# haileys/mixlab

Hardware: AMD Instinct MI355X
Metric: audio_ch_mixed_per_sec (higher is better)
Workload: dtype f32 (f64 intermediates); 1 GPU; 1024-channel Mixer + EqThree + Envelope chain (Trigger->Envelope; noise->EqThree->StereoPanner->Amplifier->Mixer), 48000 Hz f32; strips=1024, gates=toggle every 30 ticks, phase k mod 60, applied between ticks inside the batch, eq_mode=exact order: speculative time-parallel kernel, verified bit-exact, parallelism=strips sharded x1, ticks_policy=one GPU

## Files before the change

include/mixlab_gpu.h:

```cpp
#ifndef MIXLAB_GPU_H
#define MIXLAB_GPU_H

#include <stddef.h>
#include <stdint.h>

#ifdef __cplusplus
extern "C" {
#endif

#define MX_ABI_VERSION 4u

enum {
    MX_OK = 0,
    MX_ERR_INVALID = -1,
    MX_ERR_TYPE = -2,
    MX_ERR_DEVICE = -3,
    MX_ERR_NOMEM = -4,
    MX_ERR_INTERNAL = -5,
    MX_ERR_FULL = -6
};

typedef enum { MX_DISCONNECTED = 0, MX_MONO = 1, MX_STEREO = 2, MX_VIDEO = 3 } mx_line;

enum {
// ... 13 lines not shown
    MX_KIND_SOURCE_VIDEO = 13,
    MX_KIND_VIDEO_TO_RGBA = 14,
    MX_KIND_FIR = 15,
    MX_KIND_RESAMPLE = 16,
    MX_KIND_MONITOR = 17,
    MX_KIND_OUTPUT_DEVICE = 18,
    MX_KIND_COUNT = 19
};
#define MX_PROFILE_KINDS 18

enum { MX_WAVE_ON = 0, MX_WAVE_OFF = 1, MX_WAVE_SINE = 2, MX_WAVE_SQUARE = 3, MX_WAVE_TRIANGLE = 4, MX_WAVE_SAW = 5 };

typedef struct { double gain_db; double fader; uint8_t cue; uint8_t _pad[7]; } mx_mixer_channel_params;
typedef struct { double gain_lo_db, gain_mid_db, gain_hi_db; } mx_eq_three_params;
typedef struct { double attack_ms, decay_ms, sustain_amplitude, release_ms; } mx_envelope_params;
typedef struct { double amplitude, mod_depth; } mx_amplifier_params;
typedef struct { double freq; uint32_t waveform; uint32_t _pad; } mx_oscillator_params;
typedef struct { double freq_lo, freq_hi; } mx_fm_sine_params;
typedef struct { uint32_t gate_open; } mx_trigger_params;
typedef struct { int32_t a, b;  double fader; } mx_video_mixer_params;
typedef struct { int32_t use_matrix; int32_t matrix_q12[12]; } mx_video_to_rgba_params;
typedef struct { uint32_t width, height; } mx_monitor_params;
typedef struct { uint32_t width, height, queue_depth, _pad; } mx_monitor_params_ex;
typedef struct { uint32_t channels; int32_t left, right; uint32_t _pad; } mx_output_device_params;
typedef struct { uint32_t n_taps; uint32_t _pad;  } mx_fir_params;
typedef struct { uint32_t up, down, taps_per_phase, _pad;  } mx_resample_params;

typedef struct { uint32_t kind; uint32_t params_len; const void* params; } mx_node;
typedef struct { uint32_t src_node, src_port, dst_node, dst_port; } mx_edge;

#define MX_FLAG_EQ_EXACT 1u
#define MX_FLAG_EQ_FAST 4u
#define MX_FLAG_FP_CONTRACT 16u

#define MX_FLAG_OVERLAP_TAIL 8u
#define MX_FLAG_NO_FUSE 2u

typedef struct {
    uint32_t sample_rate;
    uint32_t ticks_per_second;
    uint32_t max_ticks_per_run;
    uint32_t flags;
    int32_t device;
    int32_t _pad;
    void* stream;
} mx_graph_opts;

typedef struct mx_graph mx_graph;

const char* mx_last_error(void);
uint32_t mx_abi_version(void);
int mx_device_count(void);

int mx_graph_build(const mx_node* nodes, size_t n_nodes, const mx_edge* edges, size_t n_edges,
                   const mx_graph_opts* opts, mx_graph** out);
void mx_graph_destroy(mx_graph* g);

int mx_graph_samples_per_tick(const mx_graph* g, size_t* spt);
int mx_graph_run_order(const mx_graph* g, uint32_t* order, size_t cap, size_t* n);

int mx_graph_stream(mx_graph* g, void** stream);
int mx_graph_tail_stream(mx_graph* g, void** stream);

int mx_graph_update_params(mx_graph* g, uint32_t node, const void* params, size_t params_len);

typedef struct { uint32_t node; uint32_t tick_in_run; const void* params; size_t params_len; } mx_param_event;
int mx_graph_schedule_params(mx_graph* g, uint32_t node, uint32_t tick_in_run, const void* params, size_t params_len);
int mx_graph_schedule_params_batch(mx_graph* g, const mx_param_event* events, size_t n_events);

int mx_graph_eq_spec_stats(mx_graph* g, uint64_t* chunks_run, uint64_t* chunks_repaired);
int mx_graph_eq_repair_stats(mx_graph* g, uint64_t out[8]);
int mx_graph_debug_eq_records(mx_graph* g, void** device_records, size_t* bytes);
int mx_graph_debug_tail_releases(mx_graph* g, uint64_t* gated, uint64_t* at_once);
#define MX_EQ_LAUNCH_NONE 0u
#define MX_EQ_LAUNCH_SEQUENTIAL 1u
#define MX_EQ_LAUNCH_DIRECT 2u
#define MX_EQ_LAUNCH_TILED 3u
#define MX_EQ_LAUNCH_RAGGED_TICK 4u
#define MX_EQ_LAUNCH_CONTROL_TILE 5u
#define MX_EQ_LAUNCH_SCAN 6u
int mx_graph_debug_eq_launch(mx_graph* g, uint32_t out[5]);
int mx_graph_debug_eq_env_rows(mx_graph* g, uint32_t* rows);
int mx_graph_debug_eq_lean(mx_graph* g, uint32_t* lean);
typedef struct mx_plan_node {
    int32_t pos;
    int32_t level, group;
    uint32_t slot;
    int32_t sub_key;
    uint32_t dom_num, dom_den, in_dom_num, in_dom_den;
    uint32_t elided;
    int32_t owner;
    int32_t fuse_pan, fuse_amp, fuse_trigger, fuse_env;
    uint32_t n_out;
    uint8_t out_elided[4];
    uint8_t out_dup[4];
    uint64_t out_off[4];
    uint64_t out_off2[4];
} mx_plan_node;
typedef struct mx_plan_info {
    uint64_t n_order, n_groups;
    uint64_t slab_floats;
    uint64_t zero_off, zero_floats;
    int32_t tail_first_group;
    uint32_t tail_ports;
    uint32_t tail_auto;
    uint32_t has_video;
} mx_plan_info;
int mx_graph_debug_plan(const mx_node* nodes, size_t n_nodes, const mx_edge* edges, size_t n_edges, const mx_graph_opts* opts,
                        uint32_t overlap_auto, size_t cap_frames, mx_plan_node* nodes_out, mx_plan_info* info);

int mx_graph_write_source(mx_graph* g, uint32_t node, const float* host_samples, size_t n_ticks);
int mx_graph_bind_source_device(mx_graph* g, uint32_t node, const void* device_ptr);

int mx_graph_run_ticks(mx_graph* g, uint64_t first_tick, uint32_t n_ticks);
int mx_graph_sync(mx_graph* g);

int mx_graph_read_output(mx_graph* g, uint32_t node, uint32_t port, float* host_samples, size_t n_ticks);
int mx_graph_read_output_window(mx_graph* g, uint32_t node, uint32_t port, float* host_samples, size_t first_tick_in_run, size_t n_ticks);
int mx_graph_read_output_i16(mx_graph* g, uint32_t node, uint32_t port, int16_t* host_samples, size_t n_ticks);
int mx_graph_write_source_i16(mx_graph* g, uint32_t node, const int16_t* host_samples, size_t n_ticks);

int mx_graph_output_device_ptr(mx_graph* g, uint32_t node, uint32_t port, void** device_ptr, size_t* floats_per_tick);

typedef struct { uint8_t clip, clip_status, lag_status, changed; uint32_t channels; } mx_audio_out_tick;
int mx_graph_read_audio_out(mx_graph* g, uint32_t node, uint32_t first_tick_in_run, uint32_t n_ticks, float* samples, size_t samples_cap,
                            mx_audio_out_tick* ticks, size_t* n_samples);
int mx_graph_audio_out_lag(mx_graph* g, uint32_t node);

typedef struct { uint32_t node, port; } mx_port_ref;
typedef struct { uint32_t hold_ticks; float release; } mx_meter_params;
typedef struct {
    float    peak[2];
    float    hold[2];
    double   sum_sq[2];
    uint32_t over[2];
    uint32_t frames;
    uint32_t channels;
} mx_meter_tick;
int mx_graph_set_meters(mx_graph* g, const mx_port_ref* ports, size_t n, const mx_meter_params* params);
int mx_graph_read_meters(mx_graph* g, uint32_t first_tick_in_run, uint32_t n_ticks, mx_meter_tick* dst, size_t cap);

typedef struct {
    uint32_t        n_fft;
    uint32_t        n_bands;
    const uint16_t* edges;
} mx_spectrum_params;
int mx_graph_set_spectra(mx_graph* g, const mx_port_ref* ports, size_t n, const mx_spectrum_params* params);
int mx_graph_read_spectra(mx_graph* g, uint32_t first_tick_in_run, uint32_t n_ticks, float* dst, size_t cap);
int mx_spectrum_tables(uint32_t n_fft, float* window, float* twiddle_re, float* twiddle_im);

typedef struct { uint32_t momentary_ticks; uint32_t short_ticks; } mx_loudness_params;
typedef struct {
    double   ksq[2];
    double   momentary_sq;
    double   short_sq;
    float    true_peak[2];
    uint32_t frames;
    uint32_t channels;
} mx_loudness_tick;
int mx_graph_set_loudness(mx_graph* g, const mx_port_ref* ports, size_t n, const mx_loudness_params* params);
int mx_graph_read_loudness(mx_graph* g, uint32_t first_tick_in_run, uint32_t n_ticks, mx_loudness_tick* dst, size_t cap);
int mx_loudness_tables(double rate, uint32_t frames_per_tick, double* biquads, double* carry, float* interp);
int mx_loudness_gate(const double* block_sq, const uint32_t* block_frames, size_t n_blocks, double* lufs_integrated, size_t* blocks_kept);

typedef struct { uint32_t window_ticks , grid , zoom_log2 , hop ; } mx_stereo_params;
typedef struct {
// ... 415 lines not shown
```

mixlab_amd/abi.py:

```python
from __future__ import annotations

import ctypes as C
import pathlib

import numpy as np

_PKG = pathlib.Path(__file__).resolve().parent
LIB_PATH = _PKG / "libmixlab_gpu.so"

if not LIB_PATH.exists():
    raise ImportError(
        f"{LIB_PATH} is missing: build it with `python -m mixlab_amd.build` (hipcc, gfx950). "
        "mixlab_amd has no CPU fallback."
    )

lib = C.CDLL(str(LIB_PATH))

MX_OK, MX_ERR_INVALID, MX_ERR_TYPE, MX_ERR_DEVICE, MX_ERR_NOMEM, MX_ERR_INTERNAL, MX_ERR_FULL = 0, -1, -2, -3, -4, -5, -6
MX_DISCONNECTED, MX_MONO, MX_STEREO, MX_VIDEO = 0, 1, 2, 3
(KIND_AMPLIFIER, KIND_ENVELOPE, KIND_EQ_THREE, KIND_FM_SINE, KIND_MIXER, KIND_OSCILLATOR, KIND_PLOTTER,
 KIND_STEREO_PANNER, KIND_STEREO_SPLITTER, KIND_TRIGGER, KIND_VIDEO_MIXER, KIND_SOURCE_MONO,
 KIND_SOURCE_STEREO, KIND_SOURCE_VIDEO, KIND_VIDEO_TO_RGBA, KIND_FIR, KIND_RESAMPLE, KIND_MONITOR, KIND_OUTPUT_DEVICE, KIND_COUNT) = range(20)
PROFILE_KINDS = 18
KIND_NAMES = ["amplifier", "envelope", "eq_three", "fm_sine", "mixer", "oscillator", "plotter", "stereo_panner",
# ... 9 lines not shown


class MixerChannelParams(C.Structure):
    _fields_ = [("gain_db", C.c_double), ("fader", C.c_double), ("cue", C.c_uint8), ("_pad", C.c_uint8 * 7)]


class EqThreeParams(C.Structure):
    _fields_ = [("gain_lo_db", C.c_double), ("gain_mid_db", C.c_double), ("gain_hi_db", C.c_double)]


class EnvelopeParams(C.Structure):
    _fields_ = [("attack_ms", C.c_double), ("decay_ms", C.c_double), ("sustain_amplitude", C.c_double), ("release_ms", C.c_double)]


class AmplifierParams(C.Structure):
    _fields_ = [("amplitude", C.c_double), ("mod_depth", C.c_double)]


class OscillatorParams(C.Structure):
    _fields_ = [("freq", C.c_double), ("waveform", C.c_uint32), ("_pad", C.c_uint32)]


class FmSineParams(C.Structure):
    _fields_ = [("freq_lo", C.c_double), ("freq_hi", C.c_double)]


class TriggerParams(C.Structure):
    _fields_ = [("gate_open", C.c_uint32)]


class Node(C.Structure):
    _fields_ = [("kind", C.c_uint32), ("params_len", C.c_uint32), ("params", C.c_void_p)]


class Edge(C.Structure):
    _fields_ = [("src_node", C.c_uint32), ("src_port", C.c_uint32), ("dst_node", C.c_uint32), ("dst_port", C.c_uint32)]


class GraphOpts(C.Structure):
    _fields_ = [("sample_rate", C.c_uint32), ("ticks_per_second", C.c_uint32), ("max_ticks_per_run", C.c_uint32),
                ("flags", C.c_uint32), ("device", C.c_int32), ("_pad", C.c_int32), ("stream", C.c_void_p)]


class Frame(C.Structure):
    _fields_ = [("width", C.c_uint32), ("height", C.c_uint32), ("data", C.c_void_p * 3), ("stride", C.c_int32 * 3),
                ("dur_num", C.c_int64), ("dur_den", C.c_int64), ("off_num", C.c_int64), ("off_den", C.c_int64)]


class Input(C.Structure):
    _fields_ = [("kind", C.c_int), ("samples", C.c_void_p), ("len", C.c_size_t), ("video", C.c_void_p)]


class Output(C.Structure):
    _fields_ = [("kind", C.c_int), ("samples", C.c_void_p), ("len", C.c_size_t), ("video", C.c_void_p), ("video_present", C.c_int)]


def _proto(name, restype, *argtypes):
    fn = getattr(lib, name)
    fn.restype = restype
    fn.argtypes = list(argtypes)
    return fn


_proto("mx_last_error", C.c_char_p)
_proto("mx_abi_version", C.c_uint32)
_proto("mx_device_count", C.c_int)
_proto("mx_graph_build", C.c_int, C.POINTER(Node), C.c_size_t, C.POINTER(Edge), C.c_size_t, C.POINTER(GraphOpts), C.POINTER(C.c_void_p))
_proto("mx_graph_destroy", None, C.c_void_p)
_proto("mx_graph_samples_per_tick", C.c_int, C.c_void_p, C.POINTER(C.c_size_t))
_proto("mx_graph_run_order", C.c_int, C.c_void_p, C.POINTER(C.c_uint32), C.c_size_t, C.POINTER(C.c_size_t))
_proto("mx_graph_update_params", C.c_int, C.c_void_p, C.c_uint32, C.c_void_p, C.c_size_t)
class ParamEvent(C.Structure):
    _fields_ = [("node", C.c_uint32), ("tick_in_run", C.c_uint32), ("params", C.c_void_p), ("params_len", C.c_size_t)]


_proto("mx_graph_schedule_params", C.c_int, C.c_void_p, C.c_uint32, C.c_uint32, C.c_void_p, C.c_size_t)
_proto("mx_graph_schedule_params_batch", C.c_int, C.c_void_p, C.POINTER(ParamEvent), C.c_size_t)
_proto("mx_graph_eq_spec_stats", C.c_int, C.c_void_p, C.POINTER(C.c_uint64), C.POINTER(C.c_uint64))
_proto("mx_graph_debug_eq_records", C.c_int, C.c_void_p, C.POINTER(C.c_void_p), C.POINTER(C.c_size_t))
_proto("mx_graph_debug_tail_releases", C.c_int, C.c_void_p, C.POINTER(C.c_uint64), C.POINTER(C.c_uint64))
_proto("mx_graph_debug_eq_launch", C.c_int, C.c_void_p, C.POINTER(C.c_uint32))
_proto("mx_graph_debug_eq_env_rows", C.c_int, C.c_void_p, C.POINTER(C.c_uint32))
_proto("mx_graph_debug_eq_lean", C.c_int, C.c_void_p, C.POINTER(C.c_uint32))
_proto("mx_graph_eq_repair_stats", C.c_int, C.c_void_p, C.POINTER(C.c_uint64))
PLAN_NONE = 2**64 - 1


class PlanNode(C.Structure):
    _fields_ = [("pos", C.c_int32), ("level", C.c_int32), ("group", C.c_int32), ("slot", C.c_uint32), ("sub_key", C.c_int32),
                ("dom_num", C.c_uint32), ("dom_den", C.c_uint32), ("in_dom_num", C.c_uint32), ("in_dom_den", C.c_uint32),
                ("elided", C.c_uint32), ("owner", C.c_int32),
                ("fuse_pan", C.c_int32), ("fuse_amp", C.c_int32), ("fuse_trigger", C.c_int32), ("fuse_env", C.c_int32),
                ("n_out", C.c_uint32), ("out_elided", C.c_uint8 * 4), ("out_dup", C.c_uint8 * 4),
                ("out_off", C.c_uint64 * 4), ("out_off2", C.c_uint64 * 4)]


class PlanInfo(C.Structure):
    _fields_ = [("n_order", C.c_uint64), ("n_groups", C.c_uint64), ("slab_floats", C.c_uint64), ("zero_off", C.c_uint64), ("zero_floats", C.c_uint64),
                ("tail_first_group", C.c_int32), ("tail_ports", C.c_uint32), ("tail_auto", C.c_uint32), ("has_video", C.c_uint32)]


_proto("mx_graph_debug_plan", C.c_int, C.POINTER(Node), C.c_size_t, C.POINTER(Edge), C.c_size_t, C.POINTER(GraphOpts), C.c_uint32, C.c_size_t,
       C.POINTER(PlanNode), C.POINTER(PlanInfo))
_proto("mx_graph_write_source", C.c_int, C.c_void_p, C.c_uint32, C.c_void_p, C.c_size_t)
_proto("mx_graph_bind_source_device", C.c_int, C.c_void_p, C.c_uint32, C.c_void_p)
_proto("mx_graph_run_ticks", C.c_int, C.c_void_p, C.c_uint64, C.c_uint32)
_proto("mx_graph_sync", C.c_int, C.c_void_p)
_proto("mx_graph_read_output", C.c_int, C.c_void_p, C.c_uint32, C.c_uint32, C.c_void_p, C.c_size_t)
_proto("mx_graph_read_output_window", C.c_int, C.c_void_p, C.c_uint32, C.c_uint32, C.c_void_p, C.c_size_t, C.c_size_t)
_proto("mx_graph_read_output_i16", C.c_int, C.c_void_p, C.c_uint32, C.c_uint32, C.c_void_p, C.c_size_t)
_proto("mx_graph_write_source_i16", C.c_int, C.c_void_p, C.c_uint32, C.c_void_p, C.c_size_t)
_proto("mx_graph_output_device_ptr", C.c_int, C.c_void_p, C.c_uint32, C.c_uint32, C.POINTER(C.c_void_p), C.POINTER(C.c_size_t))
_proto("mx_graph_tail_stream", C.c_int, C.c_void_p, C.POINTER(C.c_void_p))
_proto("mx_graph_stream", C.c_int, C.c_void_p, C.POINTER(C.c_void_p))
_proto("mx_graph_read_plotter", C.c_int, C.c_void_p, C.c_uint32, C.c_uint32, C.c_void_p, C.c_void_p, C.POINTER(C.c_int))
class OutputDeviceParams(C.Structure):
    _fields_ = [("channels", C.c_uint32), ("left", C.c_int32), ("right", C.c_int32), ("_pad", C.c_uint32)]


class AudioOutTick(C.Structure):
    _fields_ = [("clip", C.c_uint8), ("clip_status", C.c_uint8), ("lag_status", C.c_uint8), ("changed", C.c_uint8), ("channels", C.c_uint32)]


AUDIO_OUT_TICK_DTYPE = np.dtype([("clip", np.uint8), ("clip_status", np.uint8), ("lag_status", np.uint8), ("changed", np.uint8), ("channels", np.uint32)])
_proto("mx_graph_read_audio_out", C.c_int, C.c_void_p, C.c_uint32, C.c_uint32, C.c_uint32, C.c_void_p, C.c_size_t, C.c_void_p, C.POINTER(C.c_size_t))
_proto("mx_graph_audio_out_lag", C.c_int, C.c_void_p, C.c_uint32)
class PortRef(C.Structure):
    _fields_ = [("node", C.c_uint32), ("port", C.c_uint32)]


class MeterParams(C.Structure):
    _fields_ = [("hold_ticks", C.c_uint32), ("release", C.c_float)]


METER_TICK_DTYPE = np.dtype({"names": ["peak", "hold", "sum_sq", "over", "frames", "channels"],
                             "formats": [(np.float32, 2), (np.float32, 2), (np.float64, 2), (np.uint32, 2), np.uint32, np.uint32],
                             "offsets": [0, 8, 16, 32, 40, 44], "itemsize": 48})
_proto("mx_graph_set_meters", C.c_int, C.c_void_p, C.c_void_p, C.c_size_t, C.c_void_p)
_proto("mx_graph_read_meters", C.c_int, C.c_void_p, C.c_uint32, C.c_uint32, C.c_void_p, C.c_size_t)
class SpectrumParams(C.Structure):
    _fields_ = [("n_fft", C.c_uint32), ("n_bands", C.c_uint32), ("edges", C.POINTER(C.c_uint16))]


_proto("mx_graph_set_spectra", C.c_int, C.c_void_p, C.c_void_p, C.c_size_t, C.c_void_p)
_proto("mx_graph_read_spectra", C.c_int, C.c_void_p, C.c_uint32, C.c_uint32, C.c_void_p, C.c_size_t)
_proto("mx_spectrum_tables", C.c_int, C.c_uint32, C.c_void_p, C.c_void_p, C.c_void_p)
class LoudnessParams(C.Structure):
    _fields_ = [("momentary_ticks", C.c_uint32), ("short_ticks", C.c_uint32)]


LOUDNESS_TICK_DTYPE = np.dtype({"names": ["ksq", "momentary_sq", "short_sq", "true_peak", "frames", "channels"],
                                "formats": [(np.float64, 2), np.float64, np.float64, (np.float32, 2), np.uint32, np.uint32],
                                "offsets": [0, 16, 24, 32, 40, 44], "itemsize": 48})
_proto("mx_graph_set_loudness", C.c_int, C.c_void_p, C.c_void_p, C.c_size_t, C.c_void_p)
_proto("mx_graph_read_loudness", C.c_int, C.c_void_p, C.c_uint32, C.c_uint32, C.c_void_p, C.c_size_t)
_proto("mx_loudness_tables", C.c_int, C.c_double, C.c_uint32, C.c_void_p, C.c_void_p, C.c_void_p)
_proto("mx_loudness_gate", C.c_int, C.c_void_p, C.c_void_p, C.c_size_t, C.POINTER(C.c_double), C.POINTER(C.c_size_t))
class StereoParams(C.Structure):
    _fields_ = [("window_ticks", C.c_uint32), ("grid", C.c_uint32), ("zoom_log2", C.c_uint32), ("hop", C.c_uint32)]


STEREO_TICK_DTYPE = np.dtype({"names": ["sum_ll", "sum_rr", "sum_lr", "win_ll", "win_rr", "win_lr", "frames", "nonfinite"],
                              "formats": [np.float64] * 6 + [np.uint32] * 2,
                              "offsets": [0, 8, 16, 24, 32, 40, 48, 52], "itemsize": 56})
_proto("mx_graph_set_stereo", C.c_int, C.c_void_p, C.c_void_p, C.c_size_t, C.c_void_p)
_proto("mx_graph_read_stereo", C.c_int, C.c_void_p, C.c_uint32, C.c_uint32, C.c_void_p, C.c_size_t)
# ... 453 lines not shown
    e_arr = (Edge * max(1, len(edges)))()
    for i, e in enumerate(edges):
        e_arr[i] = Edge(*e)
    return n_arr, e_arr, keep


def debug_plan(nodes, edges, sample_rate=44100, ticks_per_second=60, max_ticks_per_run=1, flags=0, overlap_auto=1, cap_frames=0):
    n_arr, e_arr, _keep = _graph_arrays(nodes, edges)
    opts = GraphOpts(sample_rate, ticks_per_second, max_ticks_per_run, flags, -1, 0, None)
    out = (PlanNode * max(1, len(nodes)))()
    info = PlanInfo()
    check(lib.mx_graph_debug_plan(n_arr, len(nodes), e_arr, len(edges), C.byref(opts), overlap_auto, cap_frames, out, C.byref(info)))
    return list(out[: len(nodes)]), info


class Graph:

    def __init__(self, nodes, edges, sample_rate=44100, ticks_per_second=60, max_ticks_per_run=1, flags=0,
                 device=-1, stream=None):
        self._h = C.c_void_p()
        n_arr, e_arr, self._keep = _graph_arrays(nodes, edges)
        opts = GraphOpts(sample_rate, ticks_per_second, max_ticks_per_run, flags, device, 0, stream)
        check(lib.mx_graph_build(n_arr, len(nodes), e_arr, len(edges), C.byref(opts), C.byref(self._h)))
        spt = C.c_size_t()
        check(lib.mx_graph_samples_per_tick(self._h, C.byref(spt)))
        self.spt = spt.value
        self.max_ticks = max_ticks_per_run
        self.n_nodes = len(nodes)

    def close(self):
        if getattr(self, "_h", None) is not None and self._h.value:
            lib.mx_graph_destroy(self._h)
            self._h = C.c_void_p()

    def __del__(self):
        try:
            self.close()
        except Exception:
            pass

    def run_order(self):
        n = C.c_size_t()
        arr = (C.c_uint32 * max(1, self.n_nodes))()
        check(lib.mx_graph_run_order(self._h, arr, self.n_nodes, C.byref(n)))
        return list(arr[: n.value])

    def update_params(self, node, params):
        blob = params_bytes(params)
        check(lib.mx_graph_update_params(self._h, node, blob, len(blob)))

    def schedule_params(self, node, tick_in_run: int, params):
        blob = params_bytes(params)
        check(lib.mx_graph_schedule_params(self._h, node, tick_in_run, blob, len(blob)))

    def schedule_params_batch(self, events: "C.Array", n: int | None = None):
        check(lib.mx_graph_schedule_params_batch(self._h, events, len(events) if n is None else n))

    def eq_repair_stats(self) -> dict:
        v = (C.c_uint64 * 8)()
        check(lib.mx_graph_eq_repair_stats(self._h, v))
        keys = ("chunks_run", "chunks_repaired", "settled_by_comparison", "walk_steps_16", "fill_steps_16", "island_rounds", "in_order_walks", "nan_fills")
        return {k: int(x) for k, x in zip(keys, v)}

    def debug_tail_releases(self):
        a, b = C.c_uint64(), C.c_uint64()
        check(lib.mx_graph_debug_tail_releases(self._h, C.byref(a), C.byref(b)))
        return a.value, b.value

    def debug_eq_launch(self) -> dict:
        v = (C.c_uint32 * 5)()
        check(lib.mx_graph_debug_eq_launch(self._h, v))
        return {"form": EQ_LAUNCH.get(v[0], str(v[0])), "super_block": int(v[1]), "n_chunks": int(v[2]), "chunk": int(v[3]), "warm": int(v[4])}

    def debug_eq_env_rows(self) -> bool:
        v = C.c_uint32()
        check(lib.mx_graph_debug_eq_env_rows(self._h, C.byref(v)))
        return bool(v.value)

    def debug_eq_lean(self) -> dict:
        v = C.c_uint32()
        check(lib.mx_graph_debug_eq_lean(self._h, C.byref(v)))
        return {"untracked": bool(v.value & 1), "unity": bool(v.value & 2)}

    def debug_eq_records(self):
        p, n = C.c_void_p(), C.c_size_t()
        check(lib.mx_graph_debug_eq_records(self._h, C.byref(p), C.byref(n)))
        return p.value, n.value

    def eq_spec_stats(self):
        a, b = C.c_uint64(), C.c_uint64()
        check(lib.mx_graph_eq_spec_stats(self._h, C.byref(a), C.byref(b)))
        return a.value, b.value

    def write_source(self, node, samples: np.ndarray, n_ticks: int):
        a = np.ascontiguousarray(samples, dtype=np.float32)
        check(lib.mx_graph_write_source(self._h, node, a.ctypes.data_as(C.c_void_p), n_ticks))

    def bind_source_device(self, node, device_ptr: int):
        check(lib.mx_graph_bind_source_device(self._h, node, C.c_void_p(device_ptr)))

    def run_ticks(self, first_tick: int, n_ticks: int = 1):
        check(lib.mx_graph_run_ticks(self._h, first_tick, n_ticks))

    def sync(self):
        check(lib.mx_graph_sync(self._h))

    def read_output(self, node, port, n_ticks: int, stereo: bool, rate=(1, 1)) -> np.ndarray:
        out = np.empty(n_ticks * (self.spt * rate[0] // rate[1]) * (2 if stereo else 1), dtype=np.float32)
        check(lib.mx_graph_read_output(self._h, node, port, out.ctypes.data_as(C.c_void_p), n_ticks))
        return out

    def read_output_window(self, node, port, first_tick: int, n_ticks: int, stereo: bool) -> np.ndarray:
        out = np.empty(n_ticks * self.spt * (2 if stereo else 1), dtype=np.float32)
        check(lib.mx_graph_read_output_window(self._h, node, port, out.ctypes.data_as(C.c_void_p), first_tick, n_ticks))
        return out

    def read_audio_out(self, node, first_tick: int, n_ticks: int):
        n = C.c_size_t(0)
        check(lib.mx_graph_read_audio_out(self._h, node, first_tick, n_ticks, None, 0, None, C.byref(n)))
        samples = np.empty(n.value, dtype=np.float32)
        ticks = np.empty(n_ticks, dtype=AUDIO_OUT_TICK_DTYPE)
        check(lib.mx_graph_read_audio_out(self._h, node, first_tick, n_ticks, samples.ctypes.data_as(C.c_void_p), n.value,
                                          ticks.ctypes.data_as(C.c_void_p), C.byref(n)))
        return samples, ticks

    def audio_out_lag(self, node):
        check(lib.mx_graph_audio_out_lag(self._h, node))

    def set_meters(self, ports, params=MeterParams(0, 1.0)):
        ports = list(ports)
        if isinstance(params, MeterParams):
            params = [params] * len(ports)
        pa = (PortRef * max(1, len(ports)))(*[PortRef(int(n), int(p)) for (n, p) in ports])
        pr = (MeterParams * max(1, len(ports)))(*[MeterParams(q.hold_ticks, q.release) for q in params])
        check(lib.mx_graph_set_meters(self._h, pa, len(ports), pr))
        self._n_meters = len(ports)

    def read_meters(self, first_tick: int, n_ticks: int) -> np.ndarray:
        n = getattr(self, "_n_meters", 0)
        out = np.zeros((n_ticks, n), dtype=METER_TICK_DTYPE)
        check(lib.mx_graph_read_meters(self._h, first_tick, n_ticks, out.ctypes.data_as(C.c_void_p), out.size))
        return out

    def set_spectra(self, ports, n_fft: int = 2048, edges=None):
        ports = list(ports)
        if not ports:
            check(lib.mx_graph_set_spectra(self._h, None, 0, None))
            self._spectra = (0, 0)
            return
        e = np.ascontiguousarray(edges, dtype=np.uint16)
        if e.ndim != 1 or e.size < 2 or not np.array_equal(e, np.asarray(edges)):
            raise ValueError("edges: at least two bin indices that fit 16 bits")
        pa = (PortRef * len(ports))(*[PortRef(int(n), int(p)) for (n, p) in ports])
        pr = SpectrumParams(int(n_fft), e.size - 1, e.ctypes.data_as(C.POINTER(C.c_uint16)))
        check(lib.mx_graph_set_spectra(self._h, pa, len(ports), C.byref(pr)))
        self._spectra = (len(ports), e.size - 1)

    def read_spectra(self, first_tick: int, n_ticks: int) -> np.ndarray:
        n, b = getattr(self, "_spectra", (0, 0))
        out = np.zeros((n_ticks, n, 2, b), dtype=np.float32)
        check(lib.mx_graph_read_spectra(self._h, first_tick, n_ticks, out.ctypes.data_as(C.c_void_p), out.size))
        return out

    def set_loudness(self, ports, momentary_ticks: int = 24, short_ticks: int = 180):
        ports = list(ports)
        if not ports:
# ... 258 lines not shown
```

mixlab_amd/build.py:

```python
from __future__ import annotations

import concurrent.futures
import os
import pathlib
import shutil
import subprocess
import sys

PKG = pathlib.Path(__file__).resolve().parent
CSRC = PKG / "csrc"
OBJ = PKG / "build"
LIB = PKG / "libmixlab_gpu.so"

HIPCC_FLAGS = [
    "--offload-arch=gfx950", "-O3", "-std=c++17", "-fPIC",
    "-ffp-contract=off", "-fno-fast-math", "-Wall", "-Wno-unused-result",
]


def sources() -> list[pathlib.Path]:
    return sorted(list(CSRC.glob("*.hip")) + list(CSRC.glob("*.cpp")))


def headers() -> list[pathlib.Path]:
    return sorted(CSRC.glob("*.hpp")) + [PKG.parent / "include" / "mixlab_gpu.h"]


def needs_build() -> bool:
    if not LIB.exists():
        return True
    t = LIB.stat().st_mtime
    return any(p.stat().st_mtime > t for p in sources() + headers())


def _hipcc() -> str:
    hipcc = shutil.which("hipcc") or "/opt/rocm/bin/hipcc"
    if not os.path.exists(hipcc):
        raise RuntimeError("hipcc not found: cannot build libmixlab_gpu.so")
    return hipcc


def _compile_one(hipcc: str, src: pathlib.Path, obj: pathlib.Path, verbose: bool) -> None:
    cmd = [hipcc, *HIPCC_FLAGS, "-c", "-x", "hip", str(src), "-o", str(obj)]
    if verbose:
        print("[mixlab_amd.build]", " ".join(cmd), file=sys.stderr)
    subprocess.run(cmd, check=True, cwd=str(PKG))


def build(force: bool = False, verbose: bool = True) -> pathlib.Path:
    if not force and not needs_build():
        return LIB
    hipcc = _hipcc()
    OBJ.mkdir(exist_ok=True)
    hdr_t = max(p.stat().st_mtime for p in headers())
    jobs, objs = [], []
    for s in sources():
        o = OBJ / (s.name + ".o")
        objs.append(o)
        if force or not o.exists() or o.stat().st_mtime < max(s.stat().st_mtime, hdr_t):
            jobs.append((s, o))
    with concurrent.futures.ThreadPoolExecutor(max_workers=min(8, max(1, len(jobs)))) as ex:
        for f in [ex.submit(_compile_one, hipcc, s, o, verbose) for (s, o) in jobs]:
            f.result()
    tmp = LIB.with_suffix(".so.tmp")
    cmd = [hipcc, "--offload-arch=gfx950", "-shared", "-fPIC", "-o", str(tmp), *[str(o) for o in objs], "-ldl"]
    if verbose:
        print("[mixlab_amd.build]", " ".join(cmd), file=sys.stderr)
    subprocess.run(cmd, check=True, cwd=str(PKG))
    os.replace(tmp, LIB)
    return LIB


if __name__ == "__main__":
    build(force="--force" in sys.argv)
    print(LIB)
```

mixlab_amd/csrc/mx_abi.cpp:

```cpp
#include <cmath>
#include <cstring>
#include <memory>
#include <string>

#include "mx_abi_common.hpp"

using mx::Error;
using mx::Graph;

struct mx_module {
    uint32_t kind = 0;
    std::unique_ptr<Graph> g;
    std::unique_ptr<mx::VideoMixer> vm;
    uint32_t tps = 60;
    std::vector<uint8_t> in_type, out_type;
};

static thread_local std::string t_last_error;
void mx_set_last_error(const std::string& s) { t_last_error = s; }

extern "C" {

const char* mx_last_error(void) { return t_last_error.c_str(); }
uint32_t mx_abi_version(void) { return MX_ABI_VERSION; }
// ... 44 lines not shown
                r.out_off2[k] = have && L.out_off2[i][k] != SIZE_MAX ? L.out_off2[i][k] : UINT64_MAX;
            }
            nodes_out[i] = r;
        }
        if (!info) return;
        *info = mx_plan_info{};
        info->n_order = P.order.size(); info->n_groups = P.groups.size();
        info->slab_floats = L.floats; info->zero_off = L.zero_off; info->zero_floats = L.zero_floats;
        info->tail_first_group = P.tail_first; info->tail_ports = (uint32_t)P.tail_ports.size();
        info->tail_auto = P.tail_auto ? 1u : 0u; info->has_video = P.has_video ? 1u : 0u;
    });
}

void mx_graph_destroy(mx_graph* g) {
    (void)guard([&] { delete g; });
}

int mx_graph_samples_per_tick(const mx_graph* g, size_t* spt) {
    return guard([&] { REQUIRE(g && spt, "NULL argument"); *spt = g->g->spt(); });
}

int mx_graph_run_order(const mx_graph* g, uint32_t* order, size_t cap, size_t* n) {
    return guard([&] {
        REQUIRE(g && n, "NULL argument");
        const auto& o = g->g->run_order();
        *n = o.size();
        for (size_t i = 0; i < o.size() && i < cap && order; ++i) order[i] = o[i];
    });
}

int mx_graph_stream(mx_graph* g, void** stream) {
    return guard([&] { REQUIRE(g && stream, "NULL argument"); *stream = (void*)g->g->stream(); });
}
int mx_graph_tail_stream(mx_graph* g, void** stream) {
    return guard([&] { REQUIRE(g && stream, "NULL argument"); *stream = (void*)g->g->tail_stream(); });
}
int mx_graph_update_params(mx_graph* g, uint32_t node, const void* params, size_t params_len) {
    return guard([&] { REQUIRE(g, "graph is NULL"); g->g->update_params(node, params, params_len); });
}

int mx_graph_schedule_params(mx_graph* g, uint32_t node, uint32_t tick_in_run, const void* params, size_t params_len) {
    return guard([&] { REQUIRE(g, "graph is NULL"); g->g->schedule_params(node, tick_in_run, params, params_len); });
}

int mx_graph_schedule_params_batch(mx_graph* g, const mx_param_event* events, size_t n_events) {
    return guard([&] {
        REQUIRE(g, "graph is NULL");
        REQUIRE(events || !n_events, "events is NULL");
        for (size_t i = 0; i < n_events; ++i) g->g->check_schedule(events[i].node, events[i].params, events[i].params_len);
        for (size_t i = 0; i < n_events; ++i) g->g->schedule_params(events[i].node, events[i].tick_in_run, events[i].params, events[i].params_len);
    });
}

int mx_graph_eq_spec_stats(mx_graph* g, uint64_t* chunks_run, uint64_t* chunks_repaired) {
    return guard([&] {
        REQUIRE(g, "graph is NULL");
        uint64_t v[8];
        g->g->eq_spec_stats(v);
        if (chunks_run) *chunks_run = v[0];
        if (chunks_repaired) *chunks_repaired = v[1];
    });
}

int mx_graph_debug_eq_records(mx_graph* g, void** device_records, size_t* bytes) {
    return guard([&] {
        REQUIRE(g && device_records, "NULL argument");
        g->g->sync();
        *device_records = g->g->debug_eq_records(bytes);
    });
}
int mx_graph_debug_tail_releases(mx_graph* g, uint64_t* gated, uint64_t* at_once) {
    return guard([&] { REQUIRE(g, "NULL argument"); g->g->tail_releases(gated, at_once); });
}

int mx_graph_debug_eq_launch(mx_graph* g, uint32_t out[5]) {
    return guard([&] { REQUIRE(g && out, "NULL argument"); g->g->eq_launch(out); });
}

int mx_graph_debug_eq_env_rows(mx_graph* g, uint32_t* rows) {
    return guard([&] { REQUIRE(g && rows, "NULL argument"); *rows = g->g->eq_env_rows() ? 1u : 0u; });
}
int mx_graph_debug_eq_lean(mx_graph* g, uint32_t* lean) {
    return guard([&] { REQUIRE(g && lean, "NULL argument"); *lean = g->g->eq_lean(); });
}

int mx_graph_eq_repair_stats(mx_graph* g, uint64_t out[8]) {
    return guard([&] {
        REQUIRE(g, "graph is NULL");
        REQUIRE(out, "out is NULL");
        g->g->eq_spec_stats(out);
    });
}

int mx_graph_write_source(mx_graph* g, uint32_t node, const float* host_samples, size_t n_ticks) {
    return guard([&] { REQUIRE(g, "graph is NULL"); g->g->write_source(node, host_samples, n_ticks * g->g->spt()); });
}

int mx_graph_bind_source_device(mx_graph* g, uint32_t node, const void* device_ptr) {
    return guard([&] { REQUIRE(g, "graph is NULL"); g->g->bind_source(node, device_ptr); });
}

int mx_graph_run_ticks(mx_graph* g, uint64_t first_tick, uint32_t n_ticks) {
    return guard([&] {
        REQUIRE(g, "graph is NULL");
        try {
            g->g->run(first_tick * (uint64_t)g->g->spt(), g->g->spt(), n_ticks);
        } catch (...) {
            g->g->drop_schedules();
            throw;
        }
    });
}

int mx_graph_sync(mx_graph* g) {
    return guard([&] { REQUIRE(g, "graph is NULL"); g->g->sync(); });
}

int mx_graph_read_output(mx_graph* g, uint32_t node, uint32_t port, float* host_samples, size_t n_ticks) {
    return guard([&] { REQUIRE(g, "graph is NULL"); g->g->read_output(node, port, host_samples, n_ticks * g->g->spt()); });
}

int mx_graph_read_output_window(mx_graph* g, uint32_t node, uint32_t port, float* host_samples, size_t first_tick_in_run, size_t n_ticks) {
    return guard([&] {
        REQUIRE(g, "graph is NULL");
        g->g->read_output(node, port, host_samples, n_ticks * g->g->spt(), first_tick_in_run * g->g->spt());
    });
}

int mx_graph_read_output_i16(mx_graph* g, uint32_t node, uint32_t port, int16_t* host_samples, size_t n_ticks) {
    return guard([&] { REQUIRE(g, "graph is NULL"); g->g->read_output_i16(node, port, host_samples, n_ticks * g->g->spt()); });
}

int mx_graph_write_source_i16(mx_graph* g, uint32_t node, const int16_t* host_samples, size_t n_ticks) {
    return guard([&] { REQUIRE(g, "graph is NULL"); g->g->write_source_i16(node, host_samples, n_ticks * g->g->spt()); });
}

int mx_graph_output_device_ptr(mx_graph* g, uint32_t node, uint32_t port, void** device_ptr, size_t* floats_per_tick) {
    return guard([&] {
        REQUIRE(g && device_ptr, "NULL argument");
        size_t fpf = 0;
        *device_ptr = g->g->output_ptr(node, port, &fpf);
        if (floats_per_tick) *floats_per_tick = fpf;
    });
}

int mx_graph_read_audio_out(mx_graph* g, uint32_t node, uint32_t first_tick_in_run, uint32_t n_ticks, float* samples, size_t samples_cap,
                            mx_audio_out_tick* ticks, size_t* n_samples) {
    static_assert(sizeof(mx_audio_out_tick) == sizeof(mx::OutTick), "mx_audio_out_tick is the device record");
    return guard([&] {
        REQUIRE(g, "graph is NULL");
        g->g->read_audio_out(node, first_tick_in_run, n_ticks, samples, samples_cap, reinterpret_cast<mx::OutTick*>(ticks), n_samples);
    });
}

int mx_graph_audio_out_lag(mx_graph* g, uint32_t node) {
    return guard([&] { REQUIRE(g, "graph is NULL"); g->g->audio_out_lag(node); });
}

int mx_graph_set_meters(mx_graph* g, const mx_port_ref* ports, size_t n, const mx_meter_params* params) {
    return guard([&] { REQUIRE(g, "graph is NULL"); g->g->meters().set(ports, n, params); });
}

int mx_graph_read_meters(mx_graph* g, uint32_t first_tick_in_run, uint32_t n_ticks, mx_meter_tick* dst, size_t cap) {
    static_assert(sizeof(mx_meter_tick) == 48 && sizeof(mx_meter_tick) == sizeof(mx::MeterTick), "mx_meter_tick is the device record");
    static_assert(offsetof(mx_meter_tick, sum_sq) == offsetof(mx::MeterTick, sum_sq) && offsetof(mx_meter_tick, frames) == offsetof(mx::MeterTick, frames),
                  "mx_meter_tick is the device record");
// ... 495 lines not shown
```

mixlab_amd/csrc/mx_engine.cpp:

```cpp
#include <chrono>

#include "mx_engine.hpp"
#include "mx_deck.hpp"

#include <cstdio>

#include <algorithm>
#include <cmath>
#include <cstring>

namespace mx {

void hip_check(hipError_t e, const char* what) {
    if (e != hipSuccess) throw Error(MX_ERR_DEVICE, std::string(what) + ": " + hipGetErrorString(e));
}

void DevBuf::alloc(size_t n) {
    free_();
    if (n == 0) n = 256;
    hipError_t e = hipMalloc(&p, n);
    if (e == hipErrorOutOfMemory) { p = nullptr; throw Error(MX_ERR_NOMEM, "hipMalloc: out of device memory"); }
    hip_check(e, "hipMalloc");
    bytes = n;
}
void DevBuf::free_() {
    if (p) (void)hipFree(p);
    p = nullptr; bytes = 0;
}

static void toeplitz_pow_ld(long double f, uint64_t n, long double res[4]) {
    long double base[4] = {1.0L - f, f * (1.0L - f), f * f * (1.0L - f), f * f * f * (1.0L - f)};
    res[0] = 1.0L; res[1] = res[2] = res[3] = 0.0L;
    auto mul = [](const long double a[4], const long double b[4], long double c[4]) {
        long double t[4] = {0, 0, 0, 0};
        for (int i = 0; i < 4; ++i) for (int j = 0; i + j < 4; ++j) t[i + j] += a[i] * b[j];
        for (int i = 0; i < 4; ++i) c[i] = t[i];
    };
    while (n) {
        if (n & 1) mul(res, base, res);
        mul(base, base, base);
        n >>= 1;
    }
}
static void toeplitz_pow(long double f, uint64_t n, double out[4]) {
    long double r[4];
    toeplitz_pow_ld(f, n, r);
    for (int i = 0; i < 4; ++i) out[i] = (double)r[i];
}
static void toeplitz_apply_ld(const long double a[4], const long double v[4], long double y[4]) {
    for (int i = 0; i < 4; ++i) { y[i] = 0.0L; for (int k = 0; k <= i; ++k) y[i] += a[k] * v[i - k]; }
}

static inline size_t floats_per_frame(uint8_t lt) { return lt == MX_MONO ? 1 : (lt == MX_STEREO ? 2 : 0); }

static PlanEnv plan_env(size_t cap_frames) {
    const char* const ae = getenv("MX_OVERLAP_AUTO");
    PlanEnv env; env.overlap_auto = !(ae && atoi(ae) == 0); env.cap_frames = cap_frames;
    return env;
}

Graph::Graph(const mx_node* nodes, size_t n_nodes, const mx_edge* edges, size_t n_edges, const mx_graph_opts& o, size_t cap_frames_override)
    : plan_(compile_plan(nodes, n_nodes, edges, n_edges, o, plan_env(cap_frames_override))) {
    flags_ = plan_.flags; tps_ = plan_.tps; sample_rate_ = (double)plan_.sample_rate;
    spt_ = plan_.spt; tap_fpc_ = spt_; cap_frames_ = plan_.cap_frames;
    open_device(o);
    nodes_.reserve(n_nodes);
    for (size_t i = 0; i < n_nodes; ++i) {
        nodes_.emplace_back(plan_.nodes[i]);
        nodes_[i].params.assign((const uint8_t*)nodes[i].params, (const uint8_t*)nodes[i].params + nodes[i].params_len);
    }
    groups_.reserve(plan_.groups.size());
    for (const PlanGroup& g : plan_.groups) groups_.emplace_back(g);
    for (Node& n : nodes_) {
        if (n.kind == MX_KIND_VIDEO_MIXER) {
            mx_video_mixer_params p; std::memcpy(&p, n.params.data(), sizeof p);
            n.vmixer.reset(new VideoMixer(p, plan_.sample_rate, stream_));
            if (!(flags_ & MX_FLAG_NO_FUSE)) n.vmixer->set_lazy_program(n.vlazy, tps_);
        }
        if (n.kind == MX_KIND_MONITOR) {
            mx_monitor_params p; std::memcpy(&p, n.params.data(), sizeof p);
            n.mon = std::make_unique<MonitorState>();
            n.mon->scaler = std::make_shared<Scaler>(p.width, p.height, stream_);
            if (n.params.size() == sizeof(mx_monitor_params_ex)) { mx_monitor_params_ex px; std::memcpy(&px, n.params.data(), sizeof px); n.mon->depth = px.queue_depth; }
        }
        if (n.kind == MX_KIND_SOURCE_VIDEO) n.vsrc = std::make_unique<VideoSourceState>();
        if (n.kind == MX_KIND_VIDEO_TO_RGBA) n.rgba = std::make_unique<RgbaSinkState>();
        n.vout.resize(n.out_type.size());
    }
    upload_eq_tables();
    if (accept_tail()) tail_gi_ = plan_.tail_first;
    layout_slab();
    build_descriptors();
    for (Node& n : nodes_) {
        if (n.kind != MX_KIND_OUTPUT_DEVICE) continue;
        n.od = std::make_unique<OutputDeviceState>((uint32_t)(spt_ * n.in_dom_num / n.in_dom_den), od_ticks());
        n.od->update(n.params.data(), od_ticks(), stream_);
        hip_check(hipStreamSynchronize(stream_), "hipStreamSynchronize");
    }
}

void Graph::open_device(const mx_graph_opts& o) {
    if (o.device >= 0) { hip_check(hipSetDevice(o.device), "hipSetDevice"); device_ = o.device; }
    else hip_check(hipGetDevice(&device_), "hipGetDevice");
    if (o.stream) { stream_ = (hipStream_t)o.stream; own_stream_ = false; }
    else { hip_check(hipStreamCreateWithFlags(&stream_, hipStreamNonBlocking), "hipStreamCreate"); own_stream_ = true; }
    { const char* const sm = getenv("MX_SIN_MODE"); sin_mode_ = sm ? atoi(sm) : 0; }
    { const char* const gt = getenv("MX_TAIL_GATE_TEST"); gate_test_ = gt && atoi(gt); }
    { const char* const er = getenv("MX_EQ_ENV_ROWS"); eq_env_rows_ = !(er && atoi(er) == 0); }
    { const char* const el = getenv("MX_EQ_LEAN"); eq_lean_ = !(el && atoi(el) == 0); }
}

void Graph::upload_eq_tables() {
    lo_f_ = 2.0 * std::sin(3.14159265358979323846264338327950288 * 420.0 / sample_rate_);
    hi_f_ = 2.0 * std::sin(3.14159265358979323846264338327950288 * 2700.0 / sample_rate_);
    std::vector<EqScanTab> tabs(4);
    const long double fs[2] = {(long double)lo_f_, (long double)hi_f_};
    for (int v = 0; v < 4; ++v) {
        const uint64_t L = 4ull << v;
        for (int f = 0; f < 2; ++f) {
            for (int j = 0; j <= 64; ++j) toeplitz_pow(fs[f], L * (uint64_t)j, tabs[v].pw[f][j]);
            for (int k = 0; k < 6; ++k) toeplitz_pow(fs[f], L << k, tabs[v].p2[f][k]);
            const long double ff = fs[f], vsa = 1.0L / 4294967295.0L;
            const long double b[4] = {ff, ff * ff, ff * ff * ff, ff * ff * ff * ff};
            const long double c[4] = {vsa, vsa * ff, vsa * ff * ff, vsa * ff * ff * ff};
            long double sum[4] = {0, 0, 0, 0};
            for (uint64_t m = 0; m < 32; ++m) {
                long double am[4], hb[4];
                toeplitz_pow_ld(ff, m, am);
                toeplitz_apply_ld(am, b, hb);
                for (int q = 0; q < 4; ++q) tabs[v].h[f][m][q] = (double)hb[q];
                if (m < L) for (int q = 0; q < 4; ++q) sum[q] += am[q];
            }
            long double cz[4];
            toeplitz_apply_ld(sum, c, cz);
            for (int q = 0; q < 4; ++q) tabs[v].cz[f][q] = (double)cz[q];
        }
    }
    eq_tabs_.alloc(tabs.size() * sizeof(EqScanTab));
    hip_check(hipMemcpy(eq_tabs_.p, tabs.data(), tabs.size() * sizeof(EqScanTab), hipMemcpyHostToDevice), "hipMemcpy(eq tabs)");
}

bool Graph::accept_tail() {
    if (plan_.tail_first < 0) return false;
    if (plan_.tail_auto) {
        const char* const ge = getenv("MX_OVERLAP_AUTO_MAX_GB");
        const double max_gb = ge ? atof(ge) : 32.0;
        size_t free_b = 0, total_b = 0;
        if (hipMemGetInfo(&free_b, &total_b) != hipSuccess) free_b = 0;
        const double extra = (double)plan_.tail_ports.size() * (double)cap_frames_ * 8.0;
        if (extra > max_gb * 1073741824.0 || extra > (double)free_b / 4.0) return false;
    }
    tail_auto_ = plan_.tail_auto;
    hip_check(hipStreamCreateWithFlags(&tail_stream_, hipStreamNonBlocking), "hipStreamCreate(tail)");
    hip_check(hipEventCreateWithFlags(&ev_head_done_, hipEventDisableTiming), "hipEventCreate");
    for (auto& e : ev_tail_done_) hip_check(hipEventCreateWithFlags(&e, hipEventDisableTiming), "hipEventCreate");
    return true;
}

OutputDeviceState::OutputDeviceState(uint32_t frames_per_tick, size_t ticks) : frames(frames_per_tick) {
    const OutState st0{-1, -1, 0u, 0u};
    state.alloc(sizeof(OutState));
    hip_check(hipMemcpy(state.p, &st0, sizeof st0, hipMemcpyHostToDevice), "hipMemcpy(output device state)");
    rec.alloc(ticks * sizeof(OutTick));
}

void OutputDeviceState::grow(uint32_t ch, size_t ticks, hipStream_t stream) {
    if (ch <= cmax) return;
    const size_t F = frames;
    DevBuf sc; sc.alloc(F * ch * sizeof(float));
    hip_check(hipMemsetAsync(sc.p, 0, F * ch * sizeof(float), stream), "hipMemsetAsync(output device scratch)");
    if (cmax) hip_check(hipMemcpyAsync(sc.p, scratch.p, F * cmax * sizeof(float), hipMemcpyDeviceToDevice, stream), "hipMemcpyAsync(output device scratch)");
    hip_check(hipStreamSynchronize(stream), "hipStreamSynchronize");
    scratch = std::move(sc);
    out.alloc(ticks * F * ch * sizeof(float));
    part.alloc(ticks * out_route_blocks(F, ch) * sizeof(uint32_t));
    cmax = ch;
}

void OutputDeviceState::update(const void* params, size_t ticks, hipStream_t stream) {
    mx_output_device_params p; std::memcpy(&p, params, sizeof p);
    channels = p.channels;
    if (!p.channels) return;
    grow(p.channels, ticks, stream);
    if (left != p.left || right != p.right)
        hip_check(hipMemsetAsync(scratch.p, 0, (size_t)frames * cmax * sizeof(float), stream), "hipMemsetAsync(output device scratch)");
    left = p.left >= 0 && (uint32_t)p.left < p.channels ? p.left : -1;
    right = p.right >= 0 && (uint32_t)p.right < p.channels ? p.right : -1;
}

size_t OutputDeviceState::offset(uint32_t tick) const {
    size_t off = 0;
    for (const Span& sp : spans)
// ... 102 lines not shown
    prof_runs_.clear(); prof_pool_.clear();
    for (Stage& st : stage_) { if (st.done) (void)hipEventDestroy(st.done); if (st.host) (void)hipHostFree(st.host); }
    if (stream_) deck_stream_retired(stream_);
    if (own_stream_ && stream_) { video_stream_retired(stream_); multiview_stream_retired(stream_); (void)hipStreamDestroy(stream_); }
}

void Graph::layout_slab() {
    SlabLayout L = mx::layout_slab(plan_, cap_frames_, tail_gi_ >= 0);
    for (size_t i = 0; i < nodes_.size(); ++i) { nodes_[i].out_off = std::move(L.out_off[i]); nodes_[i].out_off2 = std::move(L.out_off2[i]); }
    zero_off_ = L.zero_off;
    slab_floats_ = L.floats;
    slab_.alloc(L.floats * sizeof(float));
    hip_check(hipMemsetAsync(slab_.p, 0, L.floats * sizeof(float), stream_), "hipMemsetAsync(slab)");
    hip_check(hipStreamSynchronize(stream_), "hipStreamSynchronize");
}

float* Graph::out_ptr(const Node& n, uint32_t port, uint32_t parity) const {
    const size_t fpf = n.out_dup[port] ? 1 : floats_per_frame(n.out_type[port]);
    const size_t off = fpf * (run_off_frames_ * n.dom_num / n.dom_den);
    if (n.bound && port == 0) return const_cast<float*>(n.bound) + off;
    const bool alt = parity && n.out_off2[port] != SIZE_MAX;
    return (float*)slab_.p + (alt ? n.out_off2[port] : n.out_off[port]) + off;
}
const float* Graph::in_ptr(const Node& n, uint32_t port, bool null_if_disconnected, uint32_t parity) const {
    const PortRef pr = n.in_src[port];
    if (pr.node < 0) return null_if_disconnected ? nullptr : (const float*)slab_.p + zero_off_;
    return out_ptr(nodes_[pr.node], pr.port, parity);
}

static double db_to_linear(double db) { return std::pow(10.0, db / 20.0); }

void Graph::upload_group_one(Group& g, uint32_t parity) {
    const size_t n = g.nodes.size();
    auto up = [&](DevBuf& b, const void* src, size_t bytes) {
        if (b.bytes < bytes || !b.p) b.alloc(bytes);
        if (bytes) hip_check(hipMemcpy(b.p, src, bytes, hipMemcpyHostToDevice), "hipMemcpy(desc)");
    };
    DevBuf& desc = parity ? g.desc_alt : g.desc;
    switch (g.kind) {
    case MX_KIND_AMPLIFIER: {
        std::vector<AmpDesc> d(n);
        for (size_t i = 0; i < n; ++i) {
            const Node& nd = nodes_[g.nodes[i]];
            mx_amplifier_params p; std::memcpy(&p, nd.params.data(), sizeof p);
            d[i] = AmpDesc{in_ptr(nd, 0, false, parity), in_ptr(nd, 1, true, parity), out_ptr(nd, 0, parity), p.amplitude, p.mod_depth};
        }
        up(desc, d.data(), n * sizeof(AmpDesc));
        break;
    }
    case MX_KIND_ENVELOPE: {
        std::vector<EnvDesc> d(n);
        for (size_t i = 0; i < n; ++i) {
            const Node& nd = nodes_[g.nodes[i]];
            mx_envelope_params p; std::memcpy(&p, nd.params.data(), sizeof p);
            float gate_const = 0.f; uint32_t use_const = 0;
            if (nd.fuse_trigger >= 0) {
                mx_trigger_params tp; std::memcpy(&tp, nodes_[nd.fuse_trigger].params.data(), sizeof tp);
                gate_const = tp.gate_open ? 1.0f : 0.0f; use_const = 2; g.has_gates = true;
            }
            d[i] = EnvDesc{use_const ? nullptr : in_ptr(nd, 0, false, parity), out_ptr(nd, 0, parity), gate_const, use_const,
                           EnvParams{p.attack_ms, 1.0 / p.attack_ms, 1.0 / p.decay_ms,
                                     p.sustain_amplitude, 1.0 - p.sustain_amplitude, 1.0 / p.release_ms}};
        }
        up(desc, d.data(), n * sizeof(EnvDesc));
        if (!g.state.p) { g.state.alloc(n * sizeof(EnvState)); hip_check(hipMemset(g.state.p, 0, n * sizeof(EnvState)), "hipMemset"); }
        break;
    }
    case MX_KIND_EQ_THREE: {
        std::vector<EqDesc> d(n);
        std::vector<EnvTickDesc> td(n);
        bool any_env = false;
        for (size_t i = 0; i < n; ++i) {
            const Node& nd = nodes_[g.nodes[i]];
            mx_eq_three_params p; std::memcpy(&p, nd.params.data(), sizeof p);
            EqDesc e{};
            e.in = in_ptr(nd, 0, false, parity);
            e.gain_lo = db_to_linear(p.gain_lo_db); e.gain_mid = db_to_linear(p.gain_mid_db); e.gain_hi = db_to_linear(p.gain_hi_db);
            if (nd.fuse_amp >= 0) {
                const Node& amp = nodes_[nd.fuse_amp];
                if (amp.out_dup[0]) e.flags |= MX_EQF_MONO_DUP;
                mx_amplifier_params ap; std::memcpy(&ap, amp.params.data(), sizeof ap);
                e.out = out_ptr(amp, 0, parity); e.ctl = in_ptr(amp, 1, true, parity);
                e.amp_one_minus = 1.0 - ap.mod_depth; e.amp_mod_depth = ap.mod_depth; e.amp_amplitude = ap.amplitude; e.epi = 2;
            } else if (nd.fuse_pan >= 0) {
                e.out = out_ptr(nodes_[nd.fuse_pan], 0, parity); e.epi = 1;
                if (nodes_[nd.fuse_pan].out_dup[0]) e.flags |= MX_EQF_MONO_DUP;
            } else {
                e.out = out_ptr(nd, 0, parity); e.epi = 0;
            }
            if (nd.fuse_env >= 0) {
                const Node& env = nodes_[nd.fuse_env];
                mx_envelope_params ep; std::memcpy(&ep, env.params.data(), sizeof ep);
                e.flags |= MX_EQF_ENV; e.ctl = nullptr;
                e.env = EnvParams{ep.attack_ms, 1.0 / ep.attack_ms, 1.0 / ep.decay_ms, ep.sustain_amplitude, 1.0 - ep.sustain_amplitude, 1.0 / ep.release_ms};
                if (!g.state2.p) { g.state2.alloc(n * sizeof(EnvState)); hip_check(hipMemset(g.state2.p, 0, n * sizeof(EnvState)), "hipMemset"); }
                td[i] = EnvTickDesc{e.env, e.amp_one_minus, e.amp_mod_depth, (EnvState*)g.state2.p + i};
                any_env = true; g.has_gates = true;
            }
            d[i] = e;
            const int em = eq_epilogue_mode(e.epi, e.flags, e.ctl != nullptr);
            g.eq_mode = i == 0 ? em : (g.eq_mode == em ? em : -1);
            if (nd.sub_key != 0 && nd.sub_key != 1 + em && !eq_mode_warned_) {
                eq_mode_warned_ = true;
                fprintf(stderr, "mixlab_gpu: EqThree node %u was grouped for epilogue mode %d but its descriptor says %d: the group runs the general (slower) kernel\n",
                        (unsigned)g.nodes[i], nd.sub_key - 1, em);
            }
        }
        up(desc, d.data(), n * sizeof(EqDesc));
        if (any_env) up(g.tick_desc, td.data(), n * sizeof(EnvTickDesc));
        if (!g.state.p) { g.state.alloc(n * sizeof(EqState)); hip_check(hipMemset(g.state.p, 0, n * sizeof(EqState)), "hipMemset"); }
        break;
    }
    case MX_KIND_FM_SINE: {
        std::vector<FmDesc> d(n);
        for (size_t i = 0; i < n; ++i) {
            const Node& nd = nodes_[g.nodes[i]];
            mx_fm_sine_params p; std::memcpy(&p, nd.params.data(), sizeof p);
            const double freq_amp = (p.freq_hi - p.freq_lo) / 2.0;
            const double freq_mid = p.freq_lo + freq_amp;
            d[i] = FmDesc{in_ptr(nd, 0, false, parity), out_ptr(nd, 0, parity), freq_mid, freq_amp};
        }
        up(desc, d.data(), n * sizeof(FmDesc));
        break;
    }
    case MX_KIND_MIXER: {
        size_t total = 0;
        for (uint32_t id : g.nodes) total += nodes_[id].in_type.size();
        std::vector<MixChan> ch(total ? total : 1);
        DevBuf& xb = parity ? g.extra_alt : g.extra;
        if (xb.bytes < ch.size() * sizeof(MixChan) || !xb.p) xb.alloc(ch.size() * sizeof(MixChan));
        std::vector<MixDesc> d(n);
        size_t o = 0, n_dup = 0;
        for (size_t i = 0; i < n; ++i) {
            const Node& nd = nodes_[g.nodes[i]];
            const size_t nch = nd.in_type.size();
            const mx_mixer_channel_params* p = (const mx_mixer_channel_params*)nd.params.data();
            for (size_t c = 0; c < nch; ++c) {
                mx_mixer_channel_params cp; std::memcpy(&cp, p + c, sizeof cp);
                const PortRef src = nd.in_src[c];
                const uint32_t dup = (src.node >= 0 && nodes_[src.node].out_dup[src.port]) ? 1u : 0u;
                n_dup += dup;
                ch[o + c] = MixChan{in_ptr(nd, (uint32_t)c, false, parity), cp.fader * db_to_linear(cp.gain_db), cp.cue ? 1u : 0u, dup};
            }
            d[i] = MixDesc{(const MixChan*)xb.p + o, (uint32_t)nch, 0u, out_ptr(nd, 0, parity), out_ptr(nd, 1, parity)};
            o += nch;
        }
        g.dup_mode = n_dup == 0 ? 0 : (n_dup == total ? 1 : 2);
        g.max_taps = 0;
        for (uint32_t id : g.nodes) g.max_taps = std::max<uint32_t>(g.max_taps, (uint32_t)nodes_[id].in_type.size());
        hip_check(hipMemcpy(xb.p, ch.data(), ch.size() * sizeof(MixChan), hipMemcpyHostToDevice), "hipMemcpy(mixchan)");
        up(desc, d.data(), n * sizeof(MixDesc));
        break;
    }
    case MX_KIND_OSCILLATOR: {
        std::vector<OscDesc> d(n);
        for (size_t i = 0; i < n; ++i) {
            const Node& nd = nodes_[g.nodes[i]];
            mx_oscillator_params p; std::memcpy(&p, nd.params.data(), sizeof p);
            d[i] = OscDesc{out_ptr(nd, 0, parity), out_ptr(nd, 1, parity), p.freq, p.waveform, 0u};
        }
        up(desc, d.data(), n * sizeof(OscDesc));
        break;
    }
    case MX_KIND_STEREO_PANNER: {
        std::vector<PanDesc> d(n);
        for (size_t i = 0; i < n; ++i) { const Node& nd = nodes_[g.nodes[i]]; d[i] = PanDesc{in_ptr(nd, 0, false, parity), in_ptr(nd, 1, false, parity), out_ptr(nd, 0, parity)}; }
// ... 359 lines not shown
                apply_at(from);
                sync();
                run_off_frames_ = (size_t)from * fpc;
                build_descriptors();
            }
            run_span(t0 + (uint64_t)from * fpc, fpc, from, to - from, n_calls);
            from = to;
        }
        sync();
        run_off_frames_ = 0;
        build_descriptors();
    }
    if (any_sched) {
        for (uint32_t sid : sched_nodes_) {
            Node& n = nodes_[sid];
            if (!n.gate_sched.empty()) {
                mx_trigger_params tp{}; tp.gate_open = n.gate_sched.back().second;
                std::memcpy(n.params.data(), &tp, sizeof tp);
                ++gates_version_;
                n.gate_sched.clear();
            }
            n.sched.clear();
        }
        sched_nodes_.clear();
    }
    hip_check(hipGetLastError(), "kernel launch");
    last_calls_ = n_calls;
    last_frames_per_call_ = fpc;
    for (AudioTapSet* s : taps_) s->run_ticks = s->empty() ? 0u : n_calls;
    if (prof) ++prof_runs_count_;
    if (ms_by_kind) (void)profile_collect(ms_by_kind, ms_total);
}

void Graph::run_span(uint64_t t0, size_t fpc, uint32_t call_off, uint32_t n_calls, uint32_t run_calls) {
    const size_t frames = fpc * (size_t)n_calls;
    ProfSpan* prof = nullptr;
    if (prof_this_run_) {
        if (prof_pool_.empty()) prof_pool_.push_back(std::make_unique<ProfSpan>(groups_.size()));
        prof = prof_pool_.back().get();
        prof->tail_held = prof->od = prof->od_tail = prof->meters = prof->meters_tail = false;
        hip_check(hipEventRecord(prof->begin, stream_), "hipEventRecord");
    }
    std::vector<PlotJob> jobs;
    size_t gi = 0;
    bool first_eq = true;
    for (Group& g : groups_) {
        const uint32_t n = (uint32_t)g.nodes.size();
        const size_t gf = frames * g.dom_num / g.dom_den;
        const size_t gfpc = fpc * g.dom_num / g.dom_den;
        const GateBits gates{(const uint32_t*)g.gates.p, g.gate_words, call_off};
        switch (g.kind) {
        case MX_KIND_AMPLIFIER: launch_amplifier((const AmpDesc*)desc_of(g), n, gf, stream_, fp_contract()); break;
        case MX_KIND_ENVELOPE: {
            const size_t need = envelope_scratch_bytes(n, gf);
            if (need && (g.spec.bytes < need || !g.spec.p)) { sync(); g.spec.alloc(need); }
            launch_envelope((const EnvDesc*)desc_of(g), (EnvState*)g.state.p, n, gf, gfpc, gates, t0, sample_rate_, stream_, fp_contract(), need ? g.spec.p : nullptr, need ? g.spec.bytes : 0);
            break;
        }
        case MX_KIND_EQ_THREE: {
            EqRun r{gf, gfpc, n_calls, fp_contract() ? 1u : 0u, t0, sample_rate_, 1.0 / sample_rate_, lo_f_, hi_f_, nullptr};
            uint32_t launch[5] = {MX_EQ_LAUNCH_SEQUENTIAL, 0u, 1u, (uint32_t)gf, 0u};
            if (g.state2.p) {
                const size_t need = (size_t)n * n_calls * sizeof(EnvTick);
                if (g.env_ticks.bytes < need || !g.env_ticks.p) { sync(); g.env_ticks.alloc(need); }
                launch_env_ticks((const EnvTickDesc*)g.tick_desc.p, n, gates, n_calls, gfpc, t0, sample_rate_, (EnvTick*)g.env_ticks.p, stream_, fp_contract());
                r.ticks = (const EnvTick*)g.env_ticks.p;
            }
            if (eq_exact()) {
                EqSpecPlan plan;
                if (eq_plan_spec(n, gf, gfpc, lo_f_, hi_f_, plan, g.eq_mode == 6 || g.eq_mode == 7, g.eq_mode == 4 || g.eq_mode == 5)) {
                    const size_t need = eq_spec_scratch_bytes(n, plan);
                    if (g.spec.bytes < need || !g.spec.p) { sync(); g.spec.alloc(need); }
                    if (!eq_stats_.p) { eq_stats_.alloc(8 * sizeof(uint64_t)); hip_check(hipMemset(eq_stats_.p, 0, 8 * sizeof(uint64_t)), "hipMemset"); }
                    gate_armed_ = false;
                    if (deferred_.pending) {
                        if (!gate_flag_.p) { gate_flag_.alloc(64); hip_check(hipMemset(gate_flag_.p, 0, 64), "hipMemset"); }
                        r.started = (uint32_t*)gate_flag_.p; r.started_seq = ++gate_seq_; gate_armed_ = true;
                    }
                    if (first_eq) {
                        if (!eq_rows_flag_.p) { eq_rows_flag_.alloc(64); hip_check(hipMemset(eq_rows_flag_.p, 0, 64), "hipMemset"); }
                        r.env_rows = (uint32_t*)eq_rows_flag_.p; r.env_rows_seq = ++eq_rows_seq_;
                    }
                    r.lean = eq_lean_ ? 1u : 0u;
                    const bool opens_gate = launch_eq_three_spec((const EqDesc*)desc_of(g), (EqState*)g.state.p, n, r, plan, g.eq_mode, g.spec.p, (uint64_t*)eq_stats_.p, stream_, launch, eq_env_rows_);
                    if (!opens_gate && !gate_test_) gate_armed_ = false;
                    if (deferred_.pending) flush_deferred_tail(true);
                } else {
                    void* scratch = nullptr;
                    if (eq_use_poles_split(n, gf)) {
                        const size_t need = eq_poles_scratch_bytes(n, gf);
                        if (g.spec.bytes < need || !g.spec.p) { sync(); g.spec.alloc(need); }
                        scratch = g.spec.p;
                    }
                    launch_eq_three_exact((const EqDesc*)desc_of(g), (EqState*)g.state.p, n, r, scratch, stream_);
                    launch[1] = scratch ? 2u : 1u;
                }
            } else {
                EqSplit sp{1u, 5u, 0u, 0u, gf, gf, nullptr, nullptr, nullptr};
                EqSpanPow pp{};
                eq_plan_split(n, gf, lo_f_, hi_f_, sp);
                if (sp.n_split > 1) {
                    const size_t need = (size_t)n * sp.n_split * 8 * sizeof(double) + (size_t)n * 12 * sizeof(double);
                    if (g.extra.bytes < need || !g.extra.p) { sync(); g.extra.alloc(need); }
                    sp.zbuf = (double*)g.extra.p;
                    sp.bound = sp.zbuf + (size_t)n * sp.n_split * 8;
                    toeplitz_pow((long double)lo_f_, sp.span, pp.lo);
                    toeplitz_pow((long double)hi_f_, sp.span, pp.hi);
                }
                launch_eq_three_scan((const EqDesc*)desc_of(g), (EqState*)g.state.p, n, r, (const EqScanTab*)eq_tabs_.p, sp, pp, stream_);
                launch[0] = MX_EQ_LAUNCH_SCAN; launch[2] = sp.n_split; launch[3] = (uint32_t)sp.span; launch[4] = (uint32_t)sp.warm;
            }
            if (first_eq) {
                std::copy(launch, launch + 5, eq_launch_); first_eq = false;
                if (!r.env_rows) ++eq_rows_seq_;
            }
            break;
        }
        case MX_KIND_FM_SINE: launch_fm_sine((const FmDesc*)desc_of(g), n, gf, t0, sample_rate_, stream_, sin_mode_); break;
        case MX_KIND_MIXER:
            if (overlap_this_run_ && (int)gi >= tail_gi_) {
                if ((int)gi == tail_gi_) {
                    if (deferred_.pending) flush_deferred_tail(false);
                    hip_check(hipEventRecord(ev_head_done_, stream_), "hipEventRecord");
                    deferred_.items.clear(); deferred_.outs.clear(); deferred_.taps.clear(); deferred_.parity = parity_; deferred_.prof = prof;
                    if (prof) prof->tail_held = true;
                }
                deferred_.items.push_back(TailLaunch{desc_of(g), n, g.max_taps, gf, g.dup_mode, prof ? prof->group_end[gi] : nullptr});
                if (gi + 1 == groups_.size()) deferred_.pending = true;
                ++gi;
                continue;
            }
            launch_mixer((const MixDesc*)desc_of(g), n, g.max_taps , gf, g.dup_mode, stream_);
            break;
        case MX_KIND_OSCILLATOR: launch_oscillator((const OscDesc*)desc_of(g), n, gf, t0, sample_rate_, stream_, sin_mode_); break;
        case MX_KIND_STEREO_PANNER: launch_panner((const PanDesc*)desc_of(g), n, gf, stream_); break;
        case MX_KIND_STEREO_SPLITTER: launch_splitter((const SplitDesc*)desc_of(g), n, gf, stream_); break;
        case MX_KIND_TRIGGER: launch_trigger((const TrigDesc*)desc_of(g), n, gf, gfpc, &gates, stream_); break;
        case MX_KIND_FIR: launch_fir((const FirDesc*)desc_of(g), n, g.max_taps, gf, stream_, fp_contract()); break;
        case MX_KIND_RESAMPLE:
            launch_resample((const ResampleDesc*)desc_of(g), n, g.max_taps, g.rs_tab_doubles, g.rs_win_frames, frames * g.in_dom_num / g.in_dom_den, gf,
                            t0 * g.in_dom_num / g.in_dom_den, t0 * g.dom_num / g.dom_den, stream_, g.rs_common_up, fp_contract(), g.rs_common_taps, g.rs_common_down);
            break;
        case MX_KIND_PLOTTER: {
            jobs.clear();
            for (uint32_t id : g.nodes) {
                const Node& nd = nodes_[id];
                for (uint32_t c = 0; c < n_calls; ++c) {
                    if (!nd.plot_fired[call_off + c]) continue;
                    float* stage = (float*)plot_stage_.p + (size_t)nd.plot_slot[call_off + c] * 2 * fpc;
                    jobs.push_back(PlotJob{in_ptr(nd, 0, false, parity_) + (size_t)c * 2 * fpc, stage, stage + fpc});
                }
            }
            if (!jobs.empty()) {
                PlotJob* dst = (PlotJob*)plot_jobs_.p + plot_job_off_;
                stage_upload(dst, jobs.data(), jobs.size() * sizeof(PlotJob));
                launch_plotter(dst, (uint32_t)jobs.size(), fpc, stream_);
                plot_job_off_ += jobs.size();
            }
            break;
        }
        default: break;
        }
        if (prof && group_launches(g)) hip_check(hipEventRecord(prof->group_end[gi], stream_), "hipEventRecord");
        ++gi;
    }
    if (plan_.has_video) {
// ... 267 lines not shown
bool Graph::tap_port(mx_port_ref r, TapPort& t) const {
    if (r.node >= nodes_.size() || r.port >= nodes_[r.node].out_type.size()) return false;
    const Node& nd = nodes_[r.node];
    int32_t o = (int32_t)r.node;
    while (nodes_[o].elided && nodes_[o].owner >= 0) o = nodes_[o].owner;
    t.type = nd.out_type[r.port]; t.dup = nd.out_dup[r.port]; t.elided = nd.out_elided[r.port];
    t.on_tail = tail_gi_ >= 0 && nodes_[o].group >= tail_gi_; t.dom_num = nd.dom_num; t.dom_den = nd.dom_den;
    for (uint32_t par = 0; par < 2 && !t.elided; ++par)
        t.p[par] = nd.bound && r.port == 0 ? nd.bound : (const float*)slab_.p + (par && nd.out_off2[r.port] != SIZE_MAX ? nd.out_off2[r.port] : nd.out_off[r.port]);
    return true;
}

void Graph::reupload_taps(size_t fpc) {
    for (AudioTapSet* s : taps_) if (!s->empty()) s->upload(fpc);
    tap_fpc_ = fpc;
}

void Graph::launch_tap_set(AudioTapSet& s, uint32_t n_calls, ProfSpan* prof) {
    if (s.empty()) return;
    s.begin_run(n_calls);
    const uint32_t n = s.size(), n_head = overlap_this_run_ ? s.n_head : n;
    if (n_head < n) deferred_.taps.push_back(&s);
    if (n_head) s.launch(0, n_head, parity_, stream_);
    if (!prof) return;
    if (n_head) { hip_check(hipEventRecord(prof->meters_end, stream_), "hipEventRecord"); prof->meters = true; }
    prof->meters_tail = !deferred_.taps.empty();
}

void Graph::read_output_i16(uint32_t node, uint32_t port, int16_t* host, size_t frames) {
    hip_check(hipSetDevice(device_), "hipSetDevice");
    wait_tail(-1);
    if (node >= nodes_.size() || port >= nodes_[node].out_type.size()) throw Error(MX_ERR_INVALID, "output terminal out of range");
    if (frames > cap_frames_) throw Error(MX_ERR_INVALID, "more ticks than max_ticks_per_run");
    if (frames && !host) throw Error(MX_ERR_INVALID, "host_samples is NULL");
    const Node& n = nodes_[node];
    if (n.out_elided[port]) throw Error(MX_ERR_INVALID, "port is not materialised: it only feeds a fused consumer (build with MX_FLAG_NO_FUSE to observe it)");
    const size_t cnt = floats_per_frame(n.out_type[port]) * (frames * n.dom_num / n.dom_den);
    if (!cnt) return;
    if (conv_stage_.bytes < cnt * sizeof(int16_t)) { sync(); conv_stage_.alloc(cnt * sizeof(int16_t)); }
    launch_f32_to_i16(out_ptr(n, port, parity_), (int16_t*)conv_stage_.p, cnt, n.out_dup[port] ? 1 : 0, stream_);
    hip_check(hipMemcpyAsync(host, conv_stage_.p, cnt * sizeof(int16_t), hipMemcpyDeviceToHost, stream_), "hipMemcpyAsync(D2H i16)");
    sync();
}

void Graph::write_source_i16(uint32_t node, const int16_t* host, size_t frames) {
    hip_check(hipSetDevice(device_), "hipSetDevice");
    if (node >= nodes_.size()) throw Error(MX_ERR_INVALID, "node out of range");
    Node& n = nodes_[node];
    if (n.kind != MX_KIND_SOURCE_MONO && n.kind != MX_KIND_SOURCE_STEREO) throw Error(MX_ERR_INVALID, "node is not a SOURCE_*");
    if (n.bound) throw Error(MX_ERR_INVALID, "source is bound to a caller device buffer");
    if (frames > cap_frames_) throw Error(MX_ERR_INVALID, "more ticks than max_ticks_per_run");
    if (frames && !host) throw Error(MX_ERR_INVALID, "host_samples is NULL");
    const size_t cnt = floats_per_frame(n.out_type[0]) * frames;
    if (!cnt) return;
    if (conv_stage_.bytes < cnt * sizeof(int16_t)) { sync(); conv_stage_.alloc(cnt * sizeof(int16_t)); }
    hip_check(hipMemcpyAsync(conv_stage_.p, host, cnt * sizeof(int16_t), hipMemcpyHostToDevice, stream_), "hipMemcpyAsync(H2D i16)");
    launch_i16_to_f32((const int16_t*)conv_stage_.p, out_ptr(n, 0, parity_), cnt, stream_);
    sync();
}

void* Graph::debug_eq_records(size_t* bytes) const {
    for (const Group& g : groups_)
        if (g.kind == MX_KIND_EQ_THREE && g.spec.p) { if (bytes) *bytes = g.spec.bytes; return g.spec.p; }
    if (bytes) *bytes = 0;
    return nullptr;
}

bool Graph::eq_env_rows() {
    if (!eq_rows_flag_.p || !eq_rows_seq_) return false;
    sync();
    uint32_t v = 0;
    hip_check(hipMemcpy(&v, eq_rows_flag_.p, sizeof v, hipMemcpyDeviceToHost), "hipMemcpy(eq env rows)");
    return v == eq_rows_seq_;
}

uint32_t Graph::eq_lean() {
    if (!eq_rows_flag_.p || !eq_rows_seq_) return 0u;
    sync();
    uint32_t v[3] = {0u, 0u, 0u};
    hip_check(hipMemcpy(v, eq_rows_flag_.p, sizeof v, hipMemcpyDeviceToHost), "hipMemcpy(eq lean)");
    return (v[1] == eq_rows_seq_ ? 1u : 0u) | (v[2] == eq_rows_seq_ ? 2u : 0u);
}

float* Graph::output_ptr(uint32_t node, uint32_t port, size_t* fpf, bool stream_ordered_consumer) {
    if (node >= nodes_.size() || port >= nodes_[node].out_type.size()) throw Error(MX_ERR_INVALID, "output terminal out of range");
    if (nodes_[node].out_elided[port]) throw Error(MX_ERR_INVALID, "port is not materialised: it only feeds a fused consumer (build with MX_FLAG_NO_FUSE to observe it)");
    if (nodes_[node].out_dup[port]) throw Error(MX_ERR_INVALID, "port is stored as one float per frame (L == R fused result): use mx_graph_read_output, or build with MX_FLAG_NO_FUSE");
    if (fpf) *fpf = floats_per_frame(nodes_[node].out_type[port]) * (spt_ * nodes_[node].dom_num / nodes_[node].dom_den);
    if (stream_ordered_consumer && tail_gi_ >= 0 && tail_auto_ && (nodes_[node].group >= tail_gi_ || nodes_[node].out_off2[port] != SIZE_MAX)) end_auto_tail();
    return out_ptr(nodes_[node], port, parity_);
}

int Graph::read_plotter(uint32_t node, uint32_t call, float* left, float* right) {
    if (node >= nodes_.size() || nodes_[node].kind != MX_KIND_PLOTTER) throw Error(MX_ERR_INVALID, "node is not a Plotter");
    const Node& n = nodes_[node];
    if (call >= n.plot_fired.size()) throw Error(MX_ERR_INVALID, "tick_in_run is outside the last run");
    if (!n.plot_fired[call]) return 0;
    const size_t fpc = last_frames_per_call_;
    const float* stage = (const float*)plot_stage_.p + (size_t)n.plot_slot[call] * 2 * fpc;
    hip_check(hipMemcpyAsync(left, stage, fpc * sizeof(float), hipMemcpyDeviceToHost, stream_), "hipMemcpyAsync(D2H)");
    hip_check(hipMemcpyAsync(right, stage + fpc, fpc * sizeof(float), hipMemcpyDeviceToHost, stream_), "hipMemcpyAsync(D2H)");
    sync();
    return 1;
}

}
```

mixlab_amd/csrc/mx_engine.hpp:

```cpp
#pragma once
#include <algorithm>
#include <array>
#include <atomic>
#include <functional>
#include <hip/hip_runtime.h>

#include <cstdint>
#include <memory>
#include <string>
#include <deque>
#include <vector>

#include "mx_common.hpp"
#include "mx_kernels.hpp"
#include "mx_plan.hpp"
#include "mx_taps.hpp"
#include "mx_video.hpp"
#include "mx_video_graph.hpp"

namespace mx {

struct OutputDeviceState {
    uint32_t channels = 0, cmax = 0; int32_t left = -1, right = -1; const uint32_t frames;
    DevBuf scratch;
// ... 23 lines not shown
    std::vector<uint8_t> plot_fired;
    std::vector<int32_t> plot_slot;
    using VOut = mx::VOut;
    using MonTick = MonitorState::Tick;
    std::unique_ptr<VideoMixer> vmixer;
    std::vector<VOut> vout;
    std::unique_ptr<VideoSourceState> vsrc;
    std::unique_ptr<RgbaSinkState> rgba;
    std::unique_ptr<MonitorState> mon;
    std::unique_ptr<OutputDeviceState> od;
    explicit Node(const PlanNode& p) : PlanNode(p) {}
};

struct Group : PlanGroup {
    uint32_t max_taps = 0;
    uint32_t rs_common_taps = 0, rs_common_down = 0;
    uint32_t rs_common_up = 0;
    uint32_t rs_tab_doubles = 0, rs_win_frames = 0;
    DevBuf desc;
    DevBuf desc_alt, extra_alt;
    DevBuf state;
    DevBuf extra;
    DevBuf state2;
    int dup_mode = 0;
    bool has_gates = false;
    DevBuf gates; uint32_t gate_words = 0; uint64_t gates_version = ~0ull; uint32_t gates_calls = 0;
    DevBuf tick_desc;
    DevBuf env_ticks;
    DevBuf spec;
    int eq_mode = -1;
    explicit Group(const PlanGroup& g) : PlanGroup(g) {}
};

class Graph final : public TapHost {
public:
    Graph(const mx_node* nodes, size_t n_nodes, const mx_edge* edges, size_t n_edges, const mx_graph_opts& opts,
          size_t cap_frames_override = 0);
    ~Graph();

    double sample_rate() const override { return sample_rate_; }
    size_t cap_frames() const override { return cap_frames_; }
    const std::vector<uint32_t>& run_order() const { return plan_.order; }
    hipStream_t stream() const override { return stream_; }
    uint64_t lineage() const { return lineage_; }
    int device() const override { return device_; }
    uint32_t ticks_per_second() const { return tps_; }
    hipStream_t tail_stream() { if (tail_gi_ >= 0) flush_deferred_tail(false); return tail_gi_ >= 0 ? tail_stream_ : nullptr; }
    void* debug_eq_records(size_t* bytes) const;
    void join_tail() override { if (tail_gi_ >= 0) wait_tail(-1); }
    size_t n_nodes() const { return nodes_.size(); }
    bool eq_exact() const { return (flags_ & MX_FLAG_EQ_EXACT) || !(flags_ & MX_FLAG_EQ_FAST); }
    bool fp_contract() const { return (flags_ & MX_FLAG_FP_CONTRACT) != 0; }
    const Node& node(uint32_t i) const { return nodes_.at(i); }

    void update_params(uint32_t node, const void* params, size_t len);
    void schedule_params(uint32_t node, uint32_t tick_in_run, const void* params, size_t len);
    void check_schedule(uint32_t node, const void* params, size_t len) const;
    void drop_schedules();
    void eq_spec_stats(uint64_t out[8]);
    void write_source(uint32_t node, const float* host, size_t frames);
    void bind_source(uint32_t node, const void* dev);
    void run(uint64_t t0, size_t frames_per_call, uint32_t n_calls, float* ms_by_kind = nullptr, float* ms_total = nullptr);
    void sync() override;
    void profile_enable(bool on);
    uint32_t profile_collect(float* ms_by_kind, float* ms_total);
    void read_output(uint32_t node, uint32_t port, float* host, size_t frames, size_t first_frame = 0);
    void read_audio_out(uint32_t node, uint32_t first, uint32_t n, float* samples, size_t samples_cap, OutTick* ticks, size_t* n_samples);
    void audio_out_lag(uint32_t node);
    MeterTaps& meters() { return meters_; } SpectrumTaps& spectra() { return spectra_; } LoudnessTaps& loudness() { return loudness_; }
    StereoTaps& stereo() { return stereos_; } LimiterTaps& limiters() { return limiters_; } TempoTaps& tempo() { return tempos_; } TonalityTaps& tonality() { return tonalities_; }
    bool tap_port(mx_port_ref r, TapPort& t) const override; size_t tap_fpc() const override { return tap_fpc_; }
    VideoScopeTaps& video_scopes() { return scopes_; } MultiviewTap& multiview() { return multiview_; }
    size_t spt() const override { return spt_; }
    int out_line(mx_port_ref r) const override { return r.node < nodes_.size() && r.port < nodes_[r.node].out_type.size() ? (int)nodes_[r.node].out_type[r.port] : -1; }
    const VOut& video_out(mx_port_ref r) const override { return nodes_[r.node].vout[r.port]; }
    void read_output_i16(uint32_t node, uint32_t port, int16_t* host, size_t frames);
    void write_source_i16(uint32_t node, const int16_t* host, size_t frames);
    float* output_ptr(uint32_t node, uint32_t port, size_t* floats_per_tick, bool stream_ordered_consumer = true );
    bool tail_held() const { return deferred_.pending; }
    void tail_releases(uint64_t* gated, uint64_t* at_once) const { if (gated) *gated = n_gated_; if (at_once) *at_once = n_at_once_; }
    void eq_launch(uint32_t out[5]) const { for (int k = 0; k < 5; ++k) out[k] = eq_launch_[k]; }
    bool eq_env_rows();
    uint32_t eq_lean();
    void set_tail_hook(std::function<void(hipStream_t)> hook) { tail_hook_ = std::move(hook); }
    void wait_before_next_run(hipEvent_t ev) { head_waits_.push_back(ev); }
    void forget_wait_before_next_run(hipEvent_t ev) { head_waits_.erase(std::remove(head_waits_.begin(), head_waits_.end(), ev), head_waits_.end()); }
    int read_plotter(uint32_t node, uint32_t call, float* left, float* right);
    void ensure_capacity(size_t frames);
    void adopt_state(Graph& old, const int32_t* old_of_new, size_t n);
    struct Perf { bool realtime; int lag; uint32_t tick_rate; uint64_t tick_budget_us, engine_us; };
    Perf performance_info(uint64_t* module_us, size_t cap);
    void set_input_enabled(uint32_t node, uint32_t port, bool enabled);
    void set_video_source(uint32_t node, DFrame* frame, Rational dur, Rational off, bool repeat);
    void set_video_source_band(uint32_t node, uint32_t in_w, uint32_t in_full_h, uint32_t src_row0, uint32_t slice_rows, uint32_t full_w, uint32_t full_h, uint32_t row0, uint32_t band_rows);
    void set_video_source_ring(uint32_t node, DFrame* const* frames, size_t n, Rational dur, Rational off);
    void set_video_source_key(uint32_t node, const mx_video_key_params* params);
    void set_video_source_place(uint32_t node, const mx_video_place_params* params);
    void set_video_source_grade(uint32_t node, const mx_video_grade_params* params, std::shared_ptr<const LutTables> lut);
    void set_video_source_matte(uint32_t node, const mx_video_matte_params* params);
    void queue_video_source(uint32_t node, uint64_t tick, DFrame* frame, Rational dur, Rational off);
    void check_video_queue(uint32_t node, uint64_t first_tick) const;
    void check_source_write(uint32_t node, size_t frames) const;
    float* source_feed_ptr(uint32_t node, size_t frames);
    const Node::MonTick& monitor_tick(uint32_t node, uint32_t tick_in_run);
    void monitor_consume(uint32_t node, uint32_t n_ticks);
    void read_monitor_audio_i16(uint32_t node, int16_t* host, uint32_t n_ticks);
    using MonitorLayout = MonitorState::Layout;
    MonitorLayout monitor_layout(uint32_t node);
    void read_monitor_video(uint32_t node, uint32_t first_tick, uint32_t n_ticks, uint8_t* frames, uint8_t* present);
    FrameRef video_output(uint32_t node, uint32_t port);
    void rgba_output(uint32_t node, void** dev, int32_t* stride, uint32_t* w, uint32_t* h);

private:
    struct StateLoc { void* p; size_t bytes; };
    std::vector<StateLoc> state_locs(uint32_t node) const;
    uint64_t lineage_ = next_lineage();
    static uint64_t next_lineage() { static std::atomic<uint64_t> n{0}; return ++n; }
    size_t state_bytes(uint32_t node) const;
    void open_device(const mx_graph_opts& opts);
    void upload_eq_tables();
    bool accept_tail();
    void layout_slab();
    void build_descriptors();
    void upload_group(Group& g);
    void upload_group_one(Group& g, uint32_t parity);
    void run_video_tick(uint64_t t, uint32_t tick_in_run);
    const Node& node_of_kind(uint32_t node, uint32_t kind, const char* what) const;
    void run_span(uint64_t t0, size_t fpc, uint32_t call_off, uint32_t n_calls, uint32_t run_calls);
    void apply_params(uint32_t node, const void* params, size_t len);
    size_t od_ticks() const { return std::max<size_t>(1, cap_frames_ / spt_); }
    struct ProfSpan;
    void launch_outputs(uint64_t t0, uint32_t call_off, uint32_t n_calls, ProfSpan* prof);
    void launch_tap_set(AudioTapSet& s, uint32_t n_calls, ProfSpan* prof);
    void reupload_taps(size_t fpc);
    void refresh_gates(Group& g, uint32_t run_calls);
    uint32_t trigger_of_row(const Group& g, uint32_t row) const;
    void stage_upload(void* dst, const void* src, size_t bytes);
    const float* in_ptr(const Node& n, uint32_t port, bool null_if_disconnected, uint32_t parity) const;
    float* out_ptr(const Node& n, uint32_t port, uint32_t parity) const;

    const Plan plan_;
    std::vector<Node> nodes_;
    std::vector<Group> groups_;
    uint32_t flags_ = 0;
    uint32_t tps_ = 60;
    double sample_rate_ = 44100.0;
    size_t spt_ = 735;
    size_t cap_frames_ = 735;
    int device_ = 0;
    hipStream_t stream_ = nullptr;
    bool own_stream_ = false;
    DevBuf slab_;
    int tail_gi_ = -1;
    bool eq_mode_warned_ = false;
    bool tail_auto_ = false;
    int sin_mode_ = 0;
    uint32_t parity_ = 0;
    hipStream_t tail_stream_ = nullptr;
    hipEvent_t ev_head_done_ = nullptr;
    hipEvent_t ev_tail_done_[2] = {nullptr, nullptr};
    bool tail_pending_[2] = {false, false};
    bool overlap_this_run_ = false;
    struct TailLaunch { const void* desc = nullptr; uint32_t n = 0, max_ch = 0; size_t frames = 0; int dup_mode = 0; hipEvent_t prof_ev = nullptr; };
    struct DeferredTail { bool pending = false; std::vector<TailLaunch> items; uint32_t parity = 0; ProfSpan* prof = nullptr;
                          std::vector<OutRun> outs; std::vector<AudioTapSet*> taps; } deferred_;
    std::function<void(hipStream_t)> tail_hook_;
    std::vector<hipEvent_t> head_waits_;
    uint64_t n_gated_ = 0, n_at_once_ = 0;
    DevBuf gate_flag_; uint32_t gate_seq_ = 0; bool gate_armed_ = false;
    bool gate_test_ = false;
    void flush_deferred_tail(bool gated);
    void end_auto_tail();
    void wait_tail(int parity_or_all);
    const void* desc_of(const Group& g) const { return (parity_ && g.desc_alt.p) ? g.desc_alt.p : g.desc.p; }
    size_t run_off_frames_ = 0;
    uint64_t gates_version_ = 0;
    DevBuf eq_stats_;
    uint32_t eq_launch_[5] = {MX_EQ_LAUNCH_NONE, 0, 0, 0, 0};
    bool eq_env_rows_ = true;
    bool eq_lean_ = true;
    DevBuf eq_rows_flag_; uint32_t eq_rows_seq_ = 0;
    struct Stage { void* host = nullptr; size_t cap = 0; hipEvent_t done = nullptr; bool pending = false; };
    Stage stage_[4]; uint32_t stage_next_ = 0;
    uint32_t prof_runs_count_ = 0;
    std::vector<uint32_t> sched_nodes_;
    size_t tap_fpc_ = 0;
    MeterTaps meters_{*this}; SpectrumTaps spectra_{*this}; LoudnessTaps loudness_{*this}; StereoTaps stereos_{*this}; LimiterTaps limiters_{*this}; TempoTaps tempos_{*this}; TonalityTaps tonalities_{*this};
    const std::array<AudioTapSet*, 7> taps_{&meters_, &spectra_, &loudness_, &stereos_, &limiters_, &tempos_, &tonalities_};
    VideoScopeTaps scopes_{*this}; MultiviewTap multiview_{*this};
    float perf_od_ms_ = 0.f;
    bool prof_this_run_ = false;
    size_t plot_job_off_ = 0;
    size_t zero_off_ = 0;
    size_t slab_floats_ = 0;
    double lo_f_ = 0, hi_f_ = 0;
    DevBuf eq_tabs_;
    DevBuf plot_stage_, plot_jobs_;
    DevBuf conv_stage_;
    size_t last_frames_per_call_ = 0;
    bool prof_on_ = false;
    struct ProfSpan {
        hipEvent_t begin = nullptr;
        std::vector<hipEvent_t> group_end;
        hipEvent_t video_end = nullptr, tail_begin = nullptr;
        hipEvent_t od_end = nullptr, od_tail_end = nullptr;
        hipEvent_t meters_end = nullptr, meters_tail_end = nullptr;
        bool tail_held = false, od = false, od_tail = false, meters = false, meters_tail = false;
        explicit ProfSpan(size_t n_groups);
        ProfSpan(const ProfSpan&) = delete; ProfSpan& operator=(const ProfSpan&) = delete;
        ~ProfSpan();
    };
    std::vector<std::unique_ptr<ProfSpan>> prof_runs_, prof_pool_;
    uint32_t last_calls_ = 0;
    std::vector<float> perf_group_ms_;
    float perf_total_ms_ = 0.f; uint32_t perf_calls_ = 0;
    double perf_last_lag_s_ = -1.0;
};

}
```

mixlab_amd/csrc/mx_env_math.hpp:

```cpp
#pragma once
#include "mx_kernels.hpp"

namespace mx {

__device__ __forceinline__ double ms_of_u32(uint32_t dt, double sr, double rsr) {
    const double a = (double)dt;
    double q = a * rsr;
    const double r = fma(-q, sr, a);
    q = fma(r, rsr, q);
    return q * 1000.0;
}
__device__ __forceinline__ double seq_ms(uint64_t first, uint64_t last, double sr, double rsr) {
    const uint64_t dt = last - first;
    if (dt >> 32) return (double)dt / sr * 1000.0;
    return ms_of_u32((uint32_t)dt, sr, rsr);
}
__device__ __forceinline__ double clamp01(double x) { return x > 1.0 ? 1.0 : (x < 0.0 ? 0.0 : x); }

template <bool FC> __device__ __forceinline__ double mul_add(double a, double b, double c) {
    if constexpr (FC) return __builtin_fma(a, b, c); else return a * b + c;
}
template <bool FC = false>
__device__ __forceinline__ double amp_on_ms(const EnvParams& p, double ms) {
    const double attack = p.inv_attack * ms;
    const double since_decay = ms - p.attack_ms;
    const double decay_amplitude = 1.0 - clamp01(p.inv_decay * since_decay);
    const double decay = mul_add<FC>(p.one_minus_sustain, decay_amplitude, p.sustain);
    return ms < p.attack_ms ? attack : decay;
}
__device__ __forceinline__ double amp_off_ms(const EnvParams& p, double off_amp, double ms) {
    const double release_amplitude = 1.0 - clamp01(p.inv_release * ms);
    return off_amp * release_amplitude;
}

template <bool FC = false>
__device__ __forceinline__ void env_const_gate_step(const EnvParams& p, float gate, uint64_t t0, double sr, double rsr,
                                                    uint32_t& tag, uint64_t& seq, double& off_amp) {
    if (tag != 1u) { if (gate == 1.0f) { tag = 1u; seq = t0; } }
    else if (gate == 0.0f) { off_amp = amp_on_ms<FC>(p, seq_ms(seq, t0, sr, rsr)); tag = 2u; seq = t0; }
}
template <bool FC = false>
__device__ __forceinline__ double env_amplitude(const EnvParams& p, uint32_t tag, uint64_t seq, double off_amp,
                                                uint64_t t, double sr, double rsr) {
    if (tag == 0u) return 0.0;
    const double ms = seq_ms(seq, t, sr, rsr);
    return tag == 1u ? amp_on_ms<FC>(p, ms) : amp_off_ms(p, off_amp, ms);
}

__device__ __forceinline__ bool env_saturated(const EnvParams& p, uint32_t tag, uint64_t seq, uint64_t t, double sr, double rsr) {
    if (tag == 0u) return true;
    const double ms = seq_ms(seq, t, sr, rsr);
    if (tag == 1u) return p.inv_decay > 0.0 && !(ms < p.attack_ms) && p.inv_decay * (ms - p.attack_ms) >= 1.0;
    return p.inv_release > 0.0 && p.inv_release * ms >= 1.0;
}

}
```

mixlab_amd/csrc/mx_k_eq_exact.hip:

```cpp
#include <algorithm>
#include <cmath>
#include <type_traits>

#include "mx_common.hpp"
#include "mx_k_eq_common.hpp"

namespace mx {

__device__ __forceinline__ int top_bit64(uint64_t m) { return 63 - __clzll((long long)m); }
__device__ __forceinline__ uint64_t readlane_u64(uint64_t v, int l) {
    const uint32_t lo = (uint32_t)__builtin_amdgcn_readlane((int)(uint32_t)v, l);
    const uint32_t hi = (uint32_t)__builtin_amdgcn_readlane((int)(uint32_t)(v >> 32), l);
    return ((uint64_t)hi << 32) | lo;
}
__device__ __forceinline__ double readlane_f64(double v, int l) {
    return __longlong_as_double((long long)readlane_u64((uint64_t)__double_as_longlong(v), l));
}

template <bool FC>
__global__ __launch_bounds__(256) void k_env_ticks(const EnvTickDesc* __restrict__ descs, uint32_t n_inst, GateBits gates, uint32_t n_calls,
                                                    size_t fpc, uint64_t t0, double sr, double rsr, EnvTick* __restrict__ ticks) {
    const int lane = threadIdx.x & 63;
    const uint32_t inst = blockIdx.x * 4 + (threadIdx.x >> 6);
    if (inst >= n_inst) return;
// ... 13 lines not shown
        const uint64_t R = __ballot(valid && !b_prev && b_cur);
        const uint64_t F = __ballot(valid && b_prev && !b_cur);
        auto t_of = [&](int l) { return t0 + (uint64_t)(c0 + (uint32_t)l) * (uint64_t)fpc; };
        uint32_t my_tag = tag; uint64_t my_seq = seq; double my_off = off_amp;
        const uint64_t Rle = R & le, Fle = F & le;
        if (b_cur) {
            my_tag = 1u;
            if (Rle) my_seq = t_of(top_bit64(Rle));
        } else if (Fle) {
            const int fl = top_bit64(Fle);
            const uint64_t off = t_of(fl);
            const uint64_t Rb = R & ((1ull << fl) - 1ull);
            const uint64_t on = Rb ? t_of(top_bit64(Rb)) : seq;
            my_tag = 2u; my_seq = off;
            my_off = amp_on_ms<FC>(d.p, seq_ms(on, off, sr, rsr));
        }
        if (valid) {
            const uint64_t t = t_of(lane);
            EnvTick k;
            k.seq = my_seq; k.off_amp = my_off; k.tag = my_tag;
            k.flat = env_saturated(d.p, my_tag, my_seq, t, sr, rsr) ? 1u : 0u;
            const float cc = (float)env_amplitude<FC>(d.p, my_tag, my_seq, my_off, t, sr, rsr);
            k.depth = amp_depth<FC>(d.amp_one_minus, d.amp_mod_depth, (double)cc);
            ticks[(size_t)inst * n_calls + c] = k;
        }
        const int last = n_calls - c0 >= 64u ? 63 : (int)(n_calls - c0) - 1;
        tag = (uint32_t)__builtin_amdgcn_readlane((int)my_tag, last);
        seq = readlane_u64(my_seq, last);
        off_amp = readlane_f64(my_off, last);
    }
    if (lane == 0) { d.state->tag = tag; d.state->seq = seq; d.state->off_amplitude = off_amp; }
}
void launch_env_ticks(const EnvTickDesc* d, uint32_t n, const GateBits& gates, uint32_t n_calls, size_t fpc, uint64_t t0, double sample_rate, EnvTick* ticks, hipStream_t s, bool fc) {
    if (!n || !n_calls) return;
    if (fc) hipLaunchKernelGGL(k_env_ticks<true>, dim3((n + 3) / 4), dim3(256), 0, s, d, n, gates, n_calls, fpc, t0, sample_rate, 1.0 / sample_rate, ticks);
    else hipLaunchKernelGGL(k_env_ticks<false>, dim3((n + 3) / 4), dim3(256), 0, s, d, n, gates, n_calls, fpc, t0, sample_rate, 1.0 / sample_rate, ticks);
}

struct EqChunkRec {
    double start[8];
    double end[8];
    uint32_t xmin, xmax;
    uint32_t pad[2];
};

typedef float __attribute__((ext_vector_type(4))) f4v;
typedef float __attribute__((ext_vector_type(2))) f2v;
__device__ __forceinline__ f4v ld_stream4(const float* p) { return __builtin_nontemporal_load(reinterpret_cast<const f4v*>(p)); }

enum { EQM_PLAIN = 0, EQM_AMP_CONST = 1, EQM_AMP_CTL = 2, EQM_AMP_ENV = 3 };

constexpr int EQ_BLK = 16;

struct EnvLane { double A, B, k, m0, depth; uint32_t dt0; uint32_t on; uint32_t flat; uint32_t general;
                 uint32_t k0 = 0; uint64_t t_chunk = 0;  };
__device__ __forceinline__ bool env_params_nice(const EnvParams& p) {
    auto fin = [](double v) { return v == v && fabs(v) < 1.0e300; };
    return fin(p.attack_ms) && fin(p.inv_attack) && fin(p.inv_decay) && fin(p.sustain) && fin(p.one_minus_sustain) && fin(p.inv_release) &&
           p.inv_decay >= 0.0 && p.inv_release >= 0.0;
}
__device__ __forceinline__ EnvLane env_lane_coeffs(const EnvParams& p, const EnvTick& c, uint64_t t_begin, size_t n, bool nice) {
    EnvLane e;
    e.depth = c.depth; e.flat = c.flat; e.on = c.tag == 1u ? 1u : 0u;
    const bool off = c.tag == 2u;
    e.A = e.on ? p.sustain : 0.0; e.B = e.on ? p.one_minus_sustain : (off ? c.off_amp : 0.0);
    e.k = e.on ? p.inv_decay : (off ? p.inv_release : 0.0); e.m0 = e.on ? p.attack_ms : 0.0;
    const uint64_t d0 = t_begin - c.seq;
    e.dt0 = c.tag != 0u ? (uint32_t)d0 : 0u;
    const bool off_ok = !(c.off_amp < 0.0) && (c.off_amp == c.off_amp) && !signbit(c.off_amp) && fabs(c.off_amp) < 1.0e300;
    e.general = (!nice || (c.tag != 0u && ((((d0 + n) >> 32) != 0) || (off && !off_ok)))) ? 1u : 0u;
    return e;
}
enum { ENVP_ANY = 0, ENVP_OFF = 1, ENVP_ON = 2, ENVP_ON_LATE = 3 };
template <bool FC, int PH = ENVP_ANY>
__device__ __forceinline__ float env_lane_cc(const EnvParams& p, double A, double B, double k, double m0, bool on, uint32_t dt, double sr, double rsr) {
    const double ms = ms_of_u32(dt, sr, rsr);
    const double tt = k * (PH == ENVP_OFF ? ms : ms - m0);
    const double c = __builtin_fmin(tt, 1.0);
    const double val = PH == ENVP_OFF ? B * (1.0 - c) : mul_add<FC>(B, 1.0 - c, A);
    if (PH == ENVP_OFF || PH == ENVP_ON_LATE) return (float)val;
    const double att = p.inv_attack * ms;
    return (float)(((PH == ENVP_ON || on) && ms < p.attack_ms) ? att : val);
}
template <bool FC>
__device__ __forceinline__ double env_lane_depth(const EnvParams& p, const EnvLane& e, uint32_t k, double one_minus, double mod_depth, double sr, double rsr) {
    const float cc = env_lane_cc<FC>(p, e.A, e.B, e.k, e.m0, e.on != 0u, e.dt0 + k, sr, rsr);
    return amp_depth<FC>(one_minus, mod_depth, (double)cc);
}

template <int MODE, bool STEREO, int ENVK, bool FC>
__device__ __forceinline__ void eq_spec_span(const EqDesc& d, const EqRun& r, const float* __restrict__ in, float* __restrict__ outm,
                                             const float* __restrict__ ctl, const size_t n, const EnvTick& cur, const EnvLane& el, uint64_t t,
                                             EqPoles& s, uint32_t& xmin, uint32_t& xmax) {
    const double g_lo = d.gain_lo, g_mid = d.gain_mid, g_hi = d.gain_hi, lo_f = r.lo_f, hi_f = r.hi_f;
    const double one_minus = d.amp_one_minus, mod_depth = d.amp_mod_depth, amplitude = d.amp_amplitude;
    const double depth_const = one_minus + mod_depth * 1.0;
    const double rsr = r.rsr;
    uint32_t kk = 0;
    auto fold = [&](float y, float c) -> float {
        if (MODE == EQM_PLAIN) return y;
        double depth;
        if (MODE == EQM_AMP_CONST) depth = depth_const;
        else if (MODE == EQM_AMP_CTL) depth = amp_depth<FC>(one_minus, mod_depth, (double)c);
        else if (ENVK == 1) depth = el.depth;
        else if (ENVK == 2) { depth = env_lane_depth<FC>(d.env, el, kk, one_minus, mod_depth, r.sr, rsr); ++kk; }
        else { depth = env_depth<FC>(d.env, cur, one_minus, mod_depth, t, r.sr, rsr); ++t; }
        return amp_apply(y, depth, amplitude);
    };
    auto track = [&](float x) { const uint32_t b = __float_as_uint(x); xmin = b < xmin ? b : xmin; xmax = b > xmax ? b : xmax; };
    auto put4 = [&](size_t i, const float (&v)[4]) {
        if (STEREO) {
            f4v a = {v[0], v[0], v[1], v[1]}, b = {v[2], v[2], v[3], v[3]};
            __builtin_nontemporal_store(a, reinterpret_cast<f4v*>(outm + 2 * i));
            __builtin_nontemporal_store(b, reinterpret_cast<f4v*>(outm + 2 * i + 4));
        } else {
            f4v a = {v[0], v[1], v[2], v[3]};
            __builtin_nontemporal_store(a, reinterpret_cast<f4v*>(outm + i));
        }
    };
    const size_t n_blk = n / EQ_BLK;
    f4v xa[EQ_BLK / 4], ca[EQ_BLK / 4];
    if (n_blk) {
#pragma unroll
        for (int q = 0; q < EQ_BLK / 4; ++q) { xa[q] = ld_stream4(in + 4 * q); if (MODE == EQM_AMP_CTL) ca[q] = ld_stream4(ctl + 4 * q); }
    }
    for (size_t b = 0; b < n_blk; ++b) {
        f4v xb[EQ_BLK / 4], cb[EQ_BLK / 4];
        const size_t nb = (b + 1 < n_blk ? b + 1 : b) * EQ_BLK;
#pragma unroll
        for (int q = 0; q < EQ_BLK / 4; ++q) { xb[q] = ld_stream4(in + nb + 4 * q); if (MODE == EQM_AMP_CTL) cb[q] = ld_stream4(ctl + nb + 4 * q); }
#pragma unroll
        for (int q = 0; q < EQ_BLK / 4; ++q) {
            float v[4];
#pragma unroll
            for (int e = 0; e < 4; ++e) {
                const float x = xa[q][e];
                track(x);
                v[e] = fold(eq_step<FC>(s, lo_f, hi_f, g_lo, g_mid, g_hi, x), MODE == EQM_AMP_CTL ? ca[q][e] : 0.f);
            }
            put4(b * EQ_BLK + 4 * q, v);
            __builtin_amdgcn_sched_barrier(0);
        }
#pragma unroll
        for (int q = 0; q < EQ_BLK / 4; ++q) { xa[q] = xb[q]; if (MODE == EQM_AMP_CTL) ca[q] = cb[q]; }
    }
    size_t i = n_blk * EQ_BLK;
#pragma unroll 1
    for (; i + 4 <= n; i += 4) {
        const f4v x4 = ld_stream4(in + i);
        f4v c4 = {0.f, 0.f, 0.f, 0.f};
        if (MODE == EQM_AMP_CTL) c4 = ld_stream4(ctl + i);
        float v[4];
#pragma unroll
        for (int e = 0; e < 4; ++e) { track(x4[e]); v[e] = fold(eq_step<FC>(s, lo_f, hi_f, g_lo, g_mid, g_hi, x4[e]), c4[e]); }
        put4(i, v);
    }
#pragma unroll 1
    for (; i < n; ++i) {
        const float x = in[i];
        track(x);
        const float v = fold(eq_step<FC>(s, lo_f, hi_f, g_lo, g_mid, g_hi, x), MODE == EQM_AMP_CTL ? ctl[i] : 0.f);
        if (STEREO) reinterpret_cast<float2*>(outm)[i] = make_float2(v, v); else outm[i] = v;
    }
}

template <int MODE, bool STEREO, bool FC>
__device__ __forceinline__ void eq_spec_chunk(const EqDesc& d, const EqRun& r, const EnvTick* __restrict__ ticks, const size_t begin, const size_t len,
                                              EqPoles& s, uint32_t& xmin, uint32_t& xmax) {
    const float* __restrict__ in = d.in + begin;
    float* __restrict__ outm = d.out + (STEREO ? 2 * begin : begin);
// ... 178 lines not shown
    if (wlen) {
        const float* __restrict__ in = d.in + (begin - wlen);
        f4v xa[EQ_BLK / 4];
#pragma unroll
        for (int q = 0; q < EQ_BLK / 4; ++q) xa[q] = ld_stream4(in + 4 * q);
        const size_t n_blk = wlen / EQ_BLK;
        for (size_t b = 0; b < n_blk; ++b) {
            f4v xb[EQ_BLK / 4];
            const size_t nb = (b + 1 < n_blk ? b + 1 : b) * EQ_BLK;
#pragma unroll
            for (int q = 0; q < EQ_BLK / 4; ++q) xb[q] = ld_stream4(in + nb + 4 * q);
#pragma unroll
            for (int q = 0; q < EQ_BLK / 4; ++q) {
#pragma unroll
                for (int e = 0; e < 4; ++e) { const double x = (double)xa[q][e]; pump<FC>(r.lo_f, s.lo, x); pump<FC>(r.hi_f, s.hi, x); }
            }
#pragma unroll
            for (int q = 0; q < EQ_BLK / 4; ++q) xa[q] = xb[q];
        }
        s.h0 = (double)d.in[begin - 3]; s.h1 = (double)d.in[begin - 2]; s.h2 = (double)d.in[begin - 1];
    }
    EqChunkRec* rec = recs + (size_t)inst * plan.n_chunks + j;
#pragma unroll
    for (int k = 0; k < 4; ++k) { rec->start[k] = s.lo[k]; rec->start[4 + k] = s.hi[k]; }
    uint32_t xmin = 0xffffffffu, xmax = 0u;
    const EnvTick* ticks = r.ticks ? r.ticks + (size_t)inst * r.n_calls : nullptr;
    const bool stereo = !(d.epi == 0u || (d.flags & MX_EQF_MONO_DUP));
    const int mode = d.epi != 2u ? EQM_PLAIN : ((d.flags & MX_EQF_ENV) ? EQM_AMP_ENV : (d.ctl ? EQM_AMP_CTL : EQM_AMP_CONST));
    if constexpr (KMODE >= 0) {
        eq_spec_chunk<KMODE, KSTEREO != 0, FC>(d, r, ticks, begin, len, s, xmin, xmax);
    } else {
#define MX_EQ_CASE(M) case M: if (stereo) eq_spec_chunk<M, true, FC>(d, r, ticks, begin, len, s, xmin, xmax); else eq_spec_chunk<M, false, FC>(d, r, ticks, begin, len, s, xmin, xmax); break
        switch (mode) { MX_EQ_CASE(EQM_PLAIN); MX_EQ_CASE(EQM_AMP_CONST); MX_EQ_CASE(EQM_AMP_CTL); default: MX_EQ_CASE(EQM_AMP_ENV); }
#undef MX_EQ_CASE
    }
#pragma unroll
    for (int k = 0; k < 4; ++k) { rec->end[k] = s.lo[k]; rec->end[4 + k] = s.hi[k]; }
    rec->xmin = xmin; rec->xmax = xmax;
}

typedef const float __attribute__((address_space(1)))* mx_gfp1;
typedef float __attribute__((address_space(3)))* mx_lfp3;
template <int SB> struct EqTileGeo {
    static constexpr int S = SB / 4;
    static constexpr int ROWS = 64 / S;
    static constexpr int N_INSTR = S;
    static constexpr int SHIFT = S == 8 ? 1 : 2;
    static constexpr int TILE = 64 * SB;
    static __device__ __forceinline__ int sw(int row) { return (row >> SHIFT) & (S - 1); }
};

struct EqTileCtx {
    const float* in; float* out;
    uint32_t chunk0, n_chunks, C, F;
    int lane;
    int base[8];
};

__device__ __forceinline__ int eq_row_shift(uint32_t chunk, uint32_t C) { return (int)(((chunk & 31u) * (C & 31u)) & 31u); }

template <int SB, bool ALIGN_ROWS = false>
__device__ __forceinline__ void eq_tile_bases(EqTileCtx& c) {
    typedef EqTileGeo<SB> G;
    const int s = c.lane % G::S;
#pragma unroll
    for (int k = 0; k < G::N_INSTR; ++k) {
        const int cj = G::ROWS * k + c.lane / G::S;
        const int pce = s ^ G::sw(cj);
        const long long b = (long long)(c.chunk0 + (uint32_t)cj) * (long long)c.C + 4 * pce - (ALIGN_ROWS ? eq_row_shift(c.chunk0 + (uint32_t)cj, c.C) : 0);
        c.base[k] = (int)(b > 0x3fffffffLL ? 0x3fffffffLL : b);
    }
}
template <int SB>
__device__ __forceinline__ void eq_tile_issue(const EqTileCtx& c, float* buf, int so, const float* src = nullptr ) {
    typedef EqTileGeo<SB> G;
    const float* from = src ? src : c.in;
#pragma unroll
    for (int k = 0; k < G::N_INSTR; ++k) {
        const int idx = min(max(c.base[k] + so, 0), (int)c.F - 4);
        __builtin_amdgcn_global_load_lds((mx_gfp1)(from + (size_t)(uint32_t)idx), (mx_lfp3)(buf + k * 256), 16, 0, 0);
    }
}

struct EqK { double lo_f, hi_f, g_lo, g_mid, g_hi, one_minus, mod_depth, amplitude, sr, rsr; EnvParams env; };
__device__ __forceinline__ double pin_sgpr(double v) { asm volatile("; pinned %0" : "+s"(v)); return v; }
__device__ __forceinline__ EqK eq_constants(const EqDesc& d, const EqRun& r) {
    EqK k;
    k.lo_f = pin_sgpr(r.lo_f); k.hi_f = pin_sgpr(r.hi_f);
    k.g_lo = pin_sgpr(d.gain_lo); k.g_mid = pin_sgpr(d.gain_mid); k.g_hi = pin_sgpr(d.gain_hi);
    k.one_minus = pin_sgpr(d.amp_one_minus); k.mod_depth = pin_sgpr(d.amp_mod_depth); k.amplitude = pin_sgpr(d.amp_amplitude);
    k.sr = pin_sgpr(r.sr); k.rsr = pin_sgpr(r.rsr);
    k.env.attack_ms = pin_sgpr(d.env.attack_ms); k.env.inv_attack = pin_sgpr(d.env.inv_attack); k.env.inv_decay = pin_sgpr(d.env.inv_decay);
    k.env.sustain = pin_sgpr(d.env.sustain); k.env.one_minus_sustain = pin_sgpr(d.env.one_minus_sustain); k.env.inv_release = pin_sgpr(d.env.inv_release);
    return k;
}

template <int SB, int MODE, int ENVK, bool WARM, bool FC, bool LO_ONLY = false, bool TRACK = true, bool UNITY = false>
__device__ __forceinline__ void eq_tile_compute(const EqK& K, float* buf, const int lane, const int so, const int len,
                                                const EnvTick& cur, const EnvLane& el, EqPoles& s, uint32_t& xmin, uint32_t& xmax, const float* cbuf = nullptr ) {
    const double g_lo = K.g_lo, g_mid = K.g_mid, g_hi = K.g_hi, lo_f = K.lo_f, hi_f = K.hi_f;
    const double one_minus = K.one_minus, mod_depth = K.mod_depth, amplitude = K.amplitude;
    const double depth_const = one_minus + mod_depth * 1.0;
    typedef EqTileGeo<SB> G;
    const int sw = G::sw(lane);
    f4v* row = reinterpret_cast<f4v*>(buf + lane * SB);
    f4v x4 = row[0 ^ sw];
#pragma unroll 1
    for (int pce = 0; pce < G::S; ++pce) {
        const f4v xn = row[((pce + 1) & (G::S - 1)) ^ sw];
        if (WARM ? (so + 4 * pce >= len) : (so + 4 * pce < len)) {
            const double dx[4] = {(double)x4[0], (double)x4[1], (double)x4[2], (double)x4[3]};
            if (WARM) {
#pragma unroll
                for (int e = 0; e < 4; ++e) { pump<FC>(lo_f, s.lo, dx[e]); if (!LO_ONLY) pump<FC>(hi_f, s.hi, dx[e]); }
            } else {
                const double hh[4] = {s.h0, s.h1, s.h2, dx[0]};
                f4v v, c4 = {0.f, 0.f, 0.f, 0.f};
                if (MODE == EQM_AMP_CTL) c4 = reinterpret_cast<const f4v*>(cbuf + lane * SB)[pce ^ sw];
#pragma unroll
                for (int e = 0; e < 4; ++e) {
                    if (TRACK) { const uint32_t b = __float_as_uint(x4[e]); xmin = b < xmin ? b : xmin; xmax = b > xmax ? b : xmax; }
                    const float y = eq_step_h<FC>(s, lo_f, hi_f, g_lo, g_mid, g_hi, dx[e], hh[e]);
                    if (MODE == EQM_PLAIN) v[e] = y;
                    else {
                        double depth;
                        const uint32_t kk = (uint32_t)(so + 4 * pce + e);
                        if (MODE == EQM_AMP_CONST) depth = depth_const;
                        else if (MODE == EQM_AMP_CTL) depth = amp_depth<FC>(one_minus, mod_depth, (double)c4[e]);
                        else if (ENVK == 1) depth = el.depth;
                        else if (ENVK == 2) depth = env_lane_depth<FC>(K.env, el, kk - el.k0, one_minus, mod_depth, K.sr, K.rsr);
                        else depth = env_depth<FC>(K.env, cur, one_minus, mod_depth, el.t_chunk + kk, K.sr, K.rsr);
                        v[e] = UNITY ? amp_apply_unity(y, depth) : amp_apply(y, depth, amplitude);
                    }
                }
                row[pce ^ sw] = v;
            }
            s.h0 = dx[1]; s.h1 = dx[2]; s.h2 = dx[3];
        }
        x4 = xn;
    }
}

struct EqEnvRow { double off_amp; uint32_t dtk ; uint32_t where ; };
enum { EQ_ENV_ROW_ENTRIES = 68 };
template <typename T> __device__ __forceinline__ T* eq_uniform_ptr(T* p) {
    const uint64_t v = (uint64_t)p;
    return (T*)(((uint64_t)(uint32_t)__builtin_amdgcn_readfirstlane((int)(uint32_t)(v >> 32)) << 32) | (uint32_t)__builtin_amdgcn_readfirstlane((int)(uint32_t)v));
}
__device__ __forceinline__ int eq_rank64(uint64_t m) { return (int)__builtin_amdgcn_mbcnt_hi((uint32_t)(m >> 32), __builtin_amdgcn_mbcnt_lo((uint32_t)m, 0u)); }
struct EqEnvRowPlan { int p_late, p_early, p_off; };
__device__ __forceinline__ EqEnvRowPlan eq_env_rows_plan(const EqK& K, EqEnvRow* tab, const EnvLane& el, const bool mine, const int lane) {
    const bool on = el.on != 0u;
    const bool early = on && ms_of_u32(el.dt0, K.sr, K.rsr) < K.env.attack_ms;
    const uint64_t m_late = __ballot(mine && on && !early), m_early = __ballot(mine && early), m_off = __ballot(mine && !on);
    const int n_late = __builtin_popcountll(m_late), n_early = __builtin_popcountll(m_early), n_off = __builtin_popcountll(m_off);
    const EqEnvRowPlan plan{(n_late + 1) >> 1, (n_early + 1) >> 1, (n_off + 1) >> 1};
    const int first = !on ? 2 * (plan.p_late + plan.p_early) : (early ? 2 * plan.p_late : 0);
    const int n = !on ? n_off : (early ? n_early : n_late);
    const int rank = eq_rank64(!on ? m_off : (early ? m_early : m_late));
    if (mine) {
        const EqEnvRow e{el.B, el.dt0 - el.k0, (uint32_t)(lane * 128) | ((uint32_t)EqTileGeo<32>::sw(lane) << 4)};
        tab[first + rank] = e;
        if (rank == n - 1 && (n & 1)) tab[first + rank + 1] = e;
    }
    return plan;
}
template <bool FC, int PH>
__device__ __forceinline__ const EqEnvRow* eq_env_row_passes(const EqK& K, char* cbuf, const EqEnvRow* e, const int n, const uint32_t soi, const uint32_t slot) {
    auto pass = [&](const EqEnvRow& row) {
        const float cc = PH == ENVP_OFF ? env_lane_cc<FC, ENVP_OFF>(K.env, 0.0, row.off_amp, K.env.inv_release, 0.0, false, row.dtk + soi, K.sr, K.rsr)
                                        : env_lane_cc<FC, PH>(K.env, K.env.sustain, K.env.one_minus_sustain, K.env.inv_decay, K.env.attack_ms, true, row.dtk + soi, K.sr, K.rsr);
        *reinterpret_cast<float*>(cbuf + (row.where ^ slot)) = cc;
    };
    int q = 0;
#pragma clang loop vectorize(disable) interleave(disable) unroll(disable)
    for (; q + 1 < n; q += 2, e += 4) { const EqEnvRow r0 = e[0], r1 = e[2]; pass(r0); pass(r1); }
    if (q < n) { const EqEnvRow r0 = e[0]; pass(r0); e += 2; }
    return e;
}
template <int SB, bool FC>
__device__ __forceinline__ void eq_env_rows(const EqK& K, float* cbuf, const EqEnvRow* tab, const EqEnvRowPlan& plan, const int lane, const int so) {
    static_assert(SB == 32, "a row is the 32 lanes of half a wave");
    const int i = lane & 31;
    const uint32_t soi = (uint32_t)(so + i);
    const uint32_t slot = (uint32_t)(((i >> 2) << 4) | ((i & 3) << 2));
    const EqEnvRow* e = tab + (lane >> 5);
    e = eq_env_row_passes<FC, ENVP_ON_LATE>(K, reinterpret_cast<char*>(cbuf), e, plan.p_late, soi, slot);
    e = eq_env_row_passes<FC, ENVP_ON>(K, reinterpret_cast<char*>(cbuf), e, plan.p_early, soi, slot);
    eq_env_row_passes<FC, ENVP_OFF>(K, reinterpret_cast<char*>(cbuf), e, plan.p_off, soi, slot);
}

template <int SB, int MODE, bool FC, bool OUT = true>
__device__ __forceinline__ void eq_tile_compute_range(const EqK& K, float* buf, const int lane, const int so, const int len, const int i_lo, const int i_hi,
                                                      const EnvTick& cur, const uint64_t t_chunk, EqPoles& s, uint32_t& xmin, uint32_t& xmax) {
    typedef EqTileGeo<SB> G;
    const int sw = G::sw(lane);
    f4v* row = reinterpret_cast<f4v*>(buf + lane * SB);
#pragma unroll 1
    for (int pce = 0; pce < G::S; ++pce) {
        const int base = so + 4 * pce;
        if (base + 4 > i_lo && base < i_hi && base < len) {
            f4v v = row[pce ^ sw];
#pragma unroll
            for (int e = 0; e < 4; ++e) {
                if (base + e >= i_lo && base + e < i_hi) {
                    if (OUT) {
                        const uint32_t b = __float_as_uint(v[e]); xmin = b < xmin ? b : xmin; xmax = b > xmax ? b : xmax;
                        const float y = eq_step<FC>(s, K.lo_f, K.hi_f, K.g_lo, K.g_mid, K.g_hi, v[e]);
                        const double depth = env_depth<FC>(K.env, cur, K.one_minus, K.mod_depth, t_chunk + (uint64_t)(base + e), K.sr, K.rsr);
                        v[e] = MODE == EQM_AMP_ENV ? amp_apply(y, depth, K.amplitude) : y;
                    } else {
                        const double x = (double)v[e];
                        pump<FC>(K.lo_f, s.lo, x); pump<FC>(K.hi_f, s.hi, x);
                        s.h0 = s.h1; s.h1 = s.h2; s.h2 = x;
                    }
                }
            }
            if (OUT) row[pce ^ sw] = v;
        }
    }
}

template <int SB, bool STEREO, bool RAGGED = false>
__device__ __forceinline__ void eq_tile_store(const EqTileCtx& c, const float* buf, int so) {
    typedef EqTileGeo<SB> G;
#pragma unroll
    for (int k = 0; k < G::N_INSTR; ++k) {
        const f4v o = *reinterpret_cast<const f4v*>(buf + k * 256 + c.lane * 4);
        const int cj = G::ROWS * k + c.lane / G::S;
        const uint32_t chunk = c.chunk0 + (uint32_t)cj;
        const int idx = c.base[k] + so;
        bool mine = true;
        if (RAGGED) {
            const int i = so + 4 * ((c.lane % G::S) ^ G::sw(cj)) - eq_row_shift(chunk, c.C);
            mine = i >= 0 && i + 4 <= (int)c.C;
        }
        if (mine && chunk < c.n_chunks && idx + 4 <= (int)c.F) {
            if (STEREO) {
                f4v a = {o[0], o[0], o[1], o[1]}, b = {o[2], o[2], o[3], o[3]};
                __builtin_nontemporal_store(a, reinterpret_cast<f4v*>(c.out + 2 * idx));
                __builtin_nontemporal_store(b, reinterpret_cast<f4v*>(c.out + 2 * idx + 4));
            } else {
                __builtin_nontemporal_store(o, reinterpret_cast<f4v*>(c.out + idx));
            }
        }
    }
}

enum { EQ_WPB = 4 };
template <int SB, int KMODE, int KSTEREO, bool FC, int NBUF = 2, bool RT = false, bool ROWS = false >
__global__ __launch_bounds__(64 * EQ_WPB, 4) void k_eq_three_spec_tiled(const EqDesc* __restrict__ descs, const EqState* __restrict__ states, EqRun r, EqSpecPlan plan,
                                                                         uint32_t waves_per_inst, EqChunkRec* __restrict__ recs, uint32_t n_waves) {
    extern __shared__ __attribute__((aligned(16))) float eq_tiles_all[];
    constexpr int EQ_SB = SB, EQ_TILE = EqTileGeo<SB>::TILE;
    static_assert(!ROWS || (KMODE == EQM_AMP_ENV && !RT && NBUF == 1 && SB == 32), "the row form: the whole-tick inline Envelope over one whole-line tile");
    constexpr bool LEANK = KMODE == EQM_AMP_ENV && !RT && NBUF == 1;
    constexpr bool UPTR = LEANK;
    constexpr int EQ_TILES_PER_WAVE = (NBUF == 2 || KMODE == EQM_AMP_CTL || ROWS) ? 2 : 1;
    constexpr int EQ_WAVE_FLOATS = EQ_TILES_PER_WAVE * EQ_TILE + (ROWS ? EQ_ENV_ROW_ENTRIES * (int)(sizeof(EqEnvRow) / sizeof(float)) : 0);
    const uint32_t t_enter = (uint32_t)__builtin_amdgcn_s_memtime();
    if (r.started && blockIdx.x == gridDim.x - 1 && threadIdx.x == 0) __hip_atomic_store(r.started, r.started_seq, __ATOMIC_RELAXED, __HIP_MEMORY_SCOPE_AGENT);
    const uint32_t wib = __builtin_amdgcn_readfirstlane(threadIdx.x >> 6);
    const uint32_t wave_id = blockIdx.x * EQ_WPB + wib;
    if (wave_id >= n_waves) return;
    float* const eq_tiles = eq_tiles_all + wib * EQ_WAVE_FLOATS;
    const uint32_t inst = UPTR ? (uint32_t)__builtin_amdgcn_readfirstlane((int)(wave_id / waves_per_inst)) : wave_id / waves_per_inst;
    const EqDesc& d = descs[inst];
    const EqK K = eq_constants(d, r);
    EqTileCtx c;
    c.in = d.in; c.out = d.out;
    if constexpr (UPTR) {
        c.out = eq_uniform_ptr(d.out);
    }
    c.chunk0 = (wave_id % waves_per_inst) * 64u; c.n_chunks = plan.n_chunks; c.C = plan.chunk; c.F = (uint32_t)r.frames;
    c.lane = (int)(threadIdx.x & 63u);
    eq_tile_bases<SB, RT>(c);
    const uint32_t j = c.chunk0 + (uint32_t)c.lane;
    const bool active = j < plan.n_chunks;
    const long long begin = (long long)j * c.C;
    const int len = active ? (int)((long long)c.F - begin < (long long)c.C ? (long long)c.F - begin : (long long)c.C) : 0;
    const int len0 = (int)((long long)c.F - (long long)c.chunk0 * c.C < (long long)c.C ? (long long)c.F - (long long)c.chunk0 * c.C : (long long)c.C);
    const int row_shift = RT ? eq_row_shift(j, c.C) : 0;
    const int n_warm = (int)(plan.warm / EQ_SB), n_main = (len0 + (RT ? EQ_SB - 4 : 0) + EQ_SB - 1) / EQ_SB;
    const int total = n_warm + n_main;

    EqPoles s;
#pragma unroll
    for (int k = 0; k < 4; ++k) { s.lo[k] = 0.0; s.hi[k] = 0.0; }
    s.h0 = s.h1 = s.h2 = 0.0;
    const bool from_start = begin <= (long long)plan.warm;
    const int warm_from = from_start ? -(int)begin : -(int)plan.warm;
    if (from_start) {
        const EqState& st = states[inst];
#pragma unroll
        for (int k = 0; k < 4; ++k) { s.lo[k] = st.lo[k]; s.hi[k] = st.hi[k]; }
        s.h0 = st.history[0]; s.h1 = st.history[1]; s.h2 = st.history[2];
    } else if (active) {
        eq_spec_guess<FC>(states[inst], K.lo_f, K.hi_f, d.in[begin - (long long)plan.warm], s);
    }
    uint32_t xmin = 0xffffffffu, xmax = 0u;
    const EnvTick* ticks = r.ticks ? r.ticks + (size_t)inst * r.n_calls : nullptr;
    if constexpr (UPTR) ticks = eq_uniform_ptr(ticks);
    EnvTick cur{}; EnvLane el{};
    const bool nice = env_params_nice(d.env);
    EqChunkRec* rec = UPTR ? nullptr : recs + (size_t)inst * plan.n_chunks + (active ? j : 0);
    EqChunkRec* const recs_wave = UPTR ? eq_uniform_ptr(recs + (size_t)inst * plan.n_chunks + c.chunk0) : nullptr;
    bool rows_ran = false;
    uint32_t lean_ran = 0u;

    if constexpr (NBUF == 2) eq_tile_issue<SB>(c, eq_tiles, -(int)plan.warm);
    auto begin_sb = [&](int g) -> float* {
        const int so = (g - n_warm) * EQ_SB;
        if constexpr (NBUF == 1) {
            asm volatile("s_waitcnt lgkmcnt(0)" ::: "memory");
            eq_tile_issue<SB>(c, eq_tiles, so);
            if constexpr (KMODE == EQM_AMP_CTL) { if (so >= 0) eq_tile_issue<SB>(c, eq_tiles + EQ_TILE, so, d.ctl); }
            asm volatile("s_waitcnt vmcnt(0)" ::: "memory");
            return eq_tiles;
        }
        if (g + 1 < total) eq_tile_issue<SB>(c, eq_tiles + ((g + 1) & 1) * EQ_TILE, so + EQ_SB);
        if (g + 1 < total) { if (SB == 32) asm volatile("s_waitcnt vmcnt(8)" ::: "memory"); else asm volatile("s_waitcnt vmcnt(4)" ::: "memory"); }
        else asm volatile("s_waitcnt vmcnt(0)" ::: "memory");
        return eq_tiles + (g & 1) * EQ_TILE;
    };
    const int hi_from = (active && from_start) ? warm_from : -(int)plan.warm_hi;
    int hi_min = hi_from;
#pragma unroll
    for (int m = 32; m >= 1; m >>= 1) hi_min = min(hi_min, __shfl_xor(hi_min, m, 64));
    const int n_lo = max(0, min(n_warm, n_warm + (hi_min - (EQ_SB - 1)) / EQ_SB));
    int g = 0;
    for (; g < n_lo; ++g) {
        float* buf = begin_sb(g);
        eq_tile_compute<SB, EQM_PLAIN, 0, true, FC, true>(K, buf, c.lane, (g - n_warm) * EQ_SB - row_shift, warm_from, cur, el, s, xmin, xmax);
    }
    for (; g < n_warm; ++g) {
        float* buf = begin_sb(g);
        eq_tile_compute<SB, EQM_PLAIN, 0, true, FC>(K, buf, c.lane, (g - n_warm) * EQ_SB - row_shift, warm_from, cur, el, s, xmin, xmax);
    }
    if constexpr (UPTR) { uint32_t le = active ? (uint32_t)c.lane : 0u; asm volatile("; my record %0" : "+v"(le)); rec = recs_wave + le; }
    if (!RT && active) {
#pragma unroll
        for (int k = 0; k < 4; ++k) { rec->start[k] = s.lo[k]; rec->start[4 + k] = s.hi[k]; }
    }
    if constexpr (KMODE == EQM_AMP_ENV && RT) {
        const int fpc = (int)r.fpc;
        int tick_i = 0, so0 = 0;
        auto tick_at = [&](int ti) { const size_t tk = ((size_t)begin + (size_t)ti * (size_t)fpc) / r.fpc; return ticks[tk < r.n_calls ? tk : r.n_calls - 1]; };
        const uint64_t t_chunk = r.t0 + (uint64_t)begin;
        auto load_tick = [&]() {
            so0 = tick_i * fpc;
            const EnvTick ct = tick_at(tick_i);
            el = env_lane_coeffs(K.env, ct, t_chunk + (uint64_t)so0, r.fpc, nice);
            el.k0 = (uint32_t)so0; el.t_chunk = t_chunk;
        };
        load_tick();
        {
            float* buf = begin_sb(g);
            const EnvTick cur0 = tick_at(0);
            eq_tile_compute_range<SB, KMODE, FC, false>(K, buf, c.lane, -row_shift, len > 0 ? len : 4, -EQ_SB, 0, cur0, t_chunk, s, xmin, xmax);
            if (active) {
#pragma unroll
                for (int k = 0; k < 4; ++k) { rec->start[k] = s.lo[k]; rec->start[4 + k] = s.hi[k]; }
            }
            eq_tile_compute_range<SB, KMODE, FC>(K, buf, c.lane, -row_shift, len, 0, 0x3fffffff, cur0, t_chunk, s, xmin, xmax);
            eq_tile_store<SB, KSTEREO != 0, true>(c, buf, 0);
            ++g;
        }
        while (g < total) {
            int so_g = (g - n_warm) * EQ_SB;
            const int t_end = so0 + fpc;
            if (so_g + EQ_SB <= t_end) {
                const int envk = __ballot(active && so0 < len && el.general != 0u) != 0ull ? 3 : (__ballot(active && so0 < len && el.flat == 0u) == 0ull ? 1 : 2);
                const int g_int = n_warm + t_end / EQ_SB;
                const int g_end = g_int < total ? g_int : total;
                if (envk == 1) {
                    for (; g < g_end; ++g) { float* buf = begin_sb(g); const int so = (g - n_warm) * EQ_SB; eq_tile_compute<SB, KMODE, 1, false, FC>(K, buf, c.lane, so - row_shift, len, cur, el, s, xmin, xmax); eq_tile_store<SB, KSTEREO != 0, true>(c, buf, so); }
                } else if (envk == 2) {
                    for (; g < g_end; ++g) { float* buf = begin_sb(g); const int so = (g - n_warm) * EQ_SB; eq_tile_compute<SB, KMODE, 2, false, FC>(K, buf, c.lane, so - row_shift, len, cur, el, s, xmin, xmax); eq_tile_store<SB, KSTEREO != 0, true>(c, buf, so); }
                } else {
                    const EnvTick cur3 = tick_at(tick_i);
                    for (; g < g_end; ++g) { float* buf = begin_sb(g); const int so = (g - n_warm) * EQ_SB; eq_tile_compute<SB, KMODE, 3, false, FC>(K, buf, c.lane, so - row_shift, len, cur3, el, s, xmin, xmax); eq_tile_store<SB, KSTEREO != 0, true>(c, buf, so); }
                }
            } else {
                const EnvTick now = tick_at(tick_i), nxt = tick_at(tick_i + 1);
                for (; g < total && so_g - (EQ_SB - 4) < t_end; ++g, so_g += EQ_SB) {
                    float* buf = begin_sb(g);
                    eq_tile_compute_range<SB, KMODE, FC>(K, buf, c.lane, so_g - row_shift, len, -0x3fffffff, t_end, now, t_chunk, s, xmin, xmax);
                    eq_tile_compute_range<SB, KMODE, FC>(K, buf, c.lane, so_g - row_shift, len, t_end, 0x3fffffff, nxt, t_chunk, s, xmin, xmax);
                    eq_tile_store<SB, KSTEREO != 0, true>(c, buf, so_g);
                }
                ++tick_i; load_tick();
            }
        }
    } else if constexpr (KMODE == EQM_AMP_ENV) {
        const int sb_per_tick = (int)(r.fpc / EQ_SB);
        auto lean_form = [&](const bool track, const bool unity, auto&& tick) {
            if constexpr (!LEANK) { tick(std::true_type{}, std::false_type{}); return; }
            if (track) { if (unity) tick(std::true_type{}, std::true_type{}); else tick(std::true_type{}, std::false_type{}); }
            else { if (unity) tick(std::false_type{}, std::true_type{}); else tick(std::false_type{}, std::false_type{}); }
        };
        while (g < total) {
            const int so0 = (g - n_warm) * EQ_SB;
            uint32_t jt = j;
            if constexpr (UPTR) asm volatile("; my chunk %0" : "+v"(jt));
            const long long begin_t = (long long)jt * c.C;
            const size_t tk = ((size_t)begin_t + (size_t)so0) / r.fpc;
            cur = ticks[tk < r.n_calls ? tk : r.n_calls - 1];
            const uint64_t t = r.t0 + (uint64_t)begin_t + (uint64_t)so0;
            el = env_lane_coeffs(K.env, cur, t, r.fpc, nice);
            el.k0 = (uint32_t)so0; el.t_chunk = r.t0 + (uint64_t)begin_t;
            const int envk = __ballot(active && so0 < len && el.general != 0u) != 0ull ? 3 : (__ballot(active && so0 < len && el.flat == 0u) == 0ull ? 1 : 2);
            const int g_end = g + sb_per_tick < total ? g + sb_per_tick : total;
            const bool track = !LEANK || !r.lean || __ballot(active && so0 < len && !(xmin < xmax)) != 0ull;
            const bool unity = LEANK && r.lean && K.amplitude == 1.0;
            if (envk != 3) lean_ran |= (track ? 0u : 1u) | (unity ? 2u : 0u);
            if (envk == 1) {
                lean_form(track, unity, [&](auto TR, auto UN) {
                    for (; g < g_end; ++g) { float* buf = begin_sb(g); const int so = (g - n_warm) * EQ_SB; eq_tile_compute<SB, KMODE, 1, false, FC, false, decltype(TR)::value, decltype(UN)::value>(K, buf, c.lane, so, len, cur, el, s, xmin, xmax); eq_tile_store<SB, KSTEREO != 0>(c, buf, so); }
                });
            } else if (envk == 2) {
                if constexpr (ROWS) {
                    float* const cbuf = eq_tiles + EQ_TILE;
                    EqEnvRow* const tab = reinterpret_cast<EqEnvRow*>(eq_tiles + 2 * EQ_TILE);
                    int lt = c.lane;
                    asm volatile("; my lane %0" : "+v"(lt));
                    const EqEnvRowPlan rows = eq_env_rows_plan(K, tab, el, active && so0 < len && el.flat == 0u, lt);
                    const float cc = env_lane_cc<FC>(K.env, el.A, el.B, el.k, el.m0, el.on != 0u, el.dt0, K.sr, K.rsr);
                    const f4v cc4 = {cc, cc, cc, cc};
#pragma unroll
                    for (int q = 0; q < EQ_SB / 4; ++q) reinterpret_cast<f4v*>(cbuf + lt * EQ_SB)[q] = cc4;
                    rows_ran = true;
                    lean_form(track, unity, [&](auto TR, auto UN) {
                        for (; g < g_end; ++g) {
                            const int so = (g - n_warm) * EQ_SB;
                            asm volatile("s_waitcnt lgkmcnt(0)" ::: "memory");
                            eq_tile_issue<SB>(c, eq_tiles, so);
                            eq_env_rows<SB, FC>(K, cbuf, tab, rows, lt, so);
                            asm volatile("s_waitcnt vmcnt(0)" ::: "memory");
                            eq_tile_compute<SB, EQM_AMP_CTL, 0, false, FC, false, decltype(TR)::value, decltype(UN)::value>(K, eq_tiles, c.lane, so, len, cur, el, s, xmin, xmax, cbuf);
                            eq_tile_store<SB, KSTEREO != 0>(c, eq_tiles, so);
                        }
                    });
                } else {
                    lean_form(track, unity, [&](auto TR, auto UN) {
                        for (; g < g_end; ++g) { float* buf = begin_sb(g); const int so = (g - n_warm) * EQ_SB; eq_tile_compute<SB, KMODE, 2, false, FC, false, decltype(TR)::value, decltype(UN)::value>(K, buf, c.lane, so, len, cur, el, s, xmin, xmax); eq_tile_store<SB, KSTEREO != 0>(c, buf, so); }
                    });
                }
            } else {
                for (; g < g_end; ++g) { float* buf = begin_sb(g); const int so = (g - n_warm) * EQ_SB; eq_tile_compute<SB, KMODE, 3, false, FC>(K, buf, c.lane, so, len, cur, el, s, xmin, xmax); eq_tile_store<SB, KSTEREO != 0>(c, buf, so); }
            }
        }
    } else {
        for (; g < total; ++g) {
            float* buf = begin_sb(g);
            const int so = (g - n_warm) * EQ_SB;
            eq_tile_compute<SB, KMODE, 0, false, FC>(K, buf, c.lane, so, len, cur, el, s, xmin, xmax, KMODE == EQM_AMP_CTL ? buf + EQ_TILE : nullptr);
            eq_tile_store<SB, KSTEREO != 0>(c, buf, so);
        }
    }
    if constexpr (UPTR) {
        uint32_t le = (uint32_t)c.lane;
        asm volatile("; my record %0" : "+v"(le));
        rec = recs_wave + (active ? le : 0u);
    }
    if (ROWS && rows_ran && r.env_rows && c.lane == 0) __hip_atomic_store(r.env_rows, r.env_rows_seq, __ATOMIC_RELAXED, __HIP_MEMORY_SCOPE_AGENT);
    if (LEANK && r.env_rows && c.lane == 0) {
        if (lean_ran & 1u) __hip_atomic_store(r.env_rows + 1, r.env_rows_seq, __ATOMIC_RELAXED, __HIP_MEMORY_SCOPE_AGENT);
        if (lean_ran & 2u) __hip_atomic_store(r.env_rows + 2, r.env_rows_seq, __ATOMIC_RELAXED, __HIP_MEMORY_SCOPE_AGENT);
    }
    if (active) {
#pragma unroll
        for (int k = 0; k < 4; ++k) { rec->end[k] = s.lo[k]; rec->end[4 + k] = s.hi[k]; }
        rec->xmin = xmin; rec->xmax = xmax;
        uint32_t hw = 0, xcc = 0;
        asm volatile("s_getreg_b32 %0, hwreg(HW_REG_HW_ID)" : "=s"(hw));
        asm volatile("s_getreg_b32 %0, hwreg(HW_REG_XCC_ID)" : "=s"(xcc));
        rec->pad[0] = c.lane == 0 ? t_enter : (c.lane == 1 ? hw : (c.lane == 2 ? xcc : 0u));
        rec->pad[1] = (uint32_t)__builtin_amdgcn_s_memtime();
    }
}

__device__ __forceinline__ bool same4(const double (&a)[4], const double* b) {
    bool eq = true;
#pragma unroll
    for (int k = 0; k < 4; ++k) eq = eq && (__double_as_longlong(a[k]) == __double_as_longlong(b[k]));
    return eq;
}
__device__ __forceinline__ bool same8(const double (&a)[8], const double* b) {
    bool eq = true;
#pragma unroll
    for (int k = 0; k < 8; ++k) eq = eq && (__double_as_longlong(a[k]) == __double_as_longlong(b[k]));
    return eq;
}
__device__ __forceinline__ bool all_nan4(const double (&a)[4]) { return a[0] != a[0] && a[1] != a[1] && a[2] != a[2] && a[3] != a[3]; }
__device__ __forceinline__ bool eq_all_nan(const double (&E)[8]) {
    bool a = true;
#pragma unroll
    for (int k = 0; k < 8; ++k) a = a && (E[k] != E[k]);
    return a;
}
__device__ __forceinline__ double shfl_f64(double v, int src) {
    const uint64_t u = (uint64_t)__double_as_longlong(v);
    const uint32_t lo = (uint32_t)__shfl((int)(uint32_t)u, src, 64), hi = (uint32_t)__shfl((int)(uint32_t)(u >> 32), src, 64);
    return __longlong_as_double((long long)(((uint64_t)hi << 32) | lo));
}
__device__ __forceinline__ bool grp_all(bool c, int g0) { return ((__ballot(c) >> g0) & 0xFull) == 0xFull; }
__device__ __forceinline__ void lds_handover() {
    asm volatile("" ::: "memory");
    __builtin_amdgcn_wave_barrier();
    asm volatile("" ::: "memory");
}
template <bool FC>
__device__ __forceinline__ float eq_out_of(double l, double hp, double h0, double g_lo, double g_mid, double g_hi) {
    const double h = h0 - hp;
    const double mid = h0 - (h + l);
    return band_mix<FC>(l, mid, h, g_lo, g_mid, g_hi);
}
__device__ __forceinline__ f4v eq_ld4(const float* __restrict__ p, size_t i, size_t n) {
    if (i + 4 <= n) return *reinterpret_cast<const f4v*>(p + i);
    f4v v = {0.f, 0.f, 0.f, 0.f};
    if (i < n) v[0] = p[i];
    if (i + 1 < n) v[1] = p[i + 1];
    if (i + 2 < n) v[2] = p[i + 2];
    return v;
}

template <bool FC>
struct EqBlkEmit {
    EqEpi E; double sr, rsr; uint64_t t0; size_t fpc;
    size_t left = 1; uint32_t call = 0, cur_call = 0xffffffffu; EnvTick cur{}; bool env = false;
    __device__ __forceinline__ void init(const EqDesc& d, const EqRun& r, uint32_t inst) {
        E = eq_epi_of(d, r.ticks ? r.ticks + (size_t)inst * r.n_calls : nullptr);
        sr = r.sr; rsr = r.rsr; t0 = r.t0; fpc = r.fpc ? r.fpc : 1;
        env = (E.flags & MX_EQF_ENV) && E.epi == 2u && E.ticks;
    }
    __device__ __forceinline__ void seek(size_t i) { if (env) { call = (uint32_t)(i / fpc); left = fpc - i % fpc; } }
    __device__ __forceinline__ void skip(size_t n) {
        if (!env) return;
        while (n >= left) { n -= left; ++call; left = fpc; }
        left -= n;
    }
    __device__ __forceinline__ void emit(size_t i, float y) {
        float v = y;
        if (E.epi == 2u) {
            double depth;
            if (env) {
                if (call != cur_call) { cur = E.ticks[call]; cur_call = call; }
                depth = env_depth<FC>(E.env, cur, E.amp_one_minus, E.amp_mod_depth, t0 + i, sr, rsr);
                if (--left == 0) { ++call; left = fpc; }
            } else {
                const double m = E.ctl ? (double)E.ctl[i] : 1.0;
// ... 482 lines not shown
```

mixlab_amd/csrc/mx_kernels.hpp:

```cpp
#pragma once
#include <hip/hip_runtime.h>
#include <stddef.h>
#include <stdint.h>

#include <algorithm>
#include <cmath>

namespace mx {

struct AmpDesc { const float* in; const float* ctl;  float* out; double amplitude; double mod_depth; };

struct EnvParams { double attack_ms, inv_attack, inv_decay, sustain, one_minus_sustain, inv_release; };
struct EnvDesc {
    const float* gate; float* out;
    float gate_const; uint32_t use_const;
    EnvParams p;
};
struct EnvState { uint32_t tag; uint32_t pad; uint64_t seq; double off_amplitude; };

struct GateBits { const uint32_t* bits; uint32_t words; uint32_t call_off; };
__host__ __device__ inline bool gate_bit(const GateBits& g, uint32_t inst, uint32_t call) {
    const uint32_t c = g.call_off + call;
    return (g.bits[(size_t)inst * g.words + (c >> 5)] >> (c & 31)) & 1u;
}

struct EnvTick { uint64_t seq; double off_amp; double depth; uint32_t tag; uint32_t flat; };
struct EnvTickDesc { EnvParams p; double amp_one_minus, amp_mod_depth; EnvState* state; };

enum { MX_EQF_MONO_DUP = 1u, MX_EQF_ENV = 2u };
struct EqDesc {
    const float* in; float* out; double gain_lo, gain_mid, gain_hi;
    const float* ctl; double amp_one_minus, amp_mod_depth, amp_amplitude; uint32_t epi; uint32_t flags;
    EnvParams env;
};
struct EqState { double lo[4]; double hi[4]; double history[3]; double pad; };

struct EqScanTab { double pw[2][65][4]; double p2[2][6][4]; double h[2][32][4]; double cz[2][4]; };

struct EqSplit { uint32_t n_split; uint32_t l2_pre; uint32_t stream_out ; uint32_t pad; size_t span; size_t warm; double* zbuf ; double* bound ; EnvState* env_snap ; };
struct EqSpanPow { double lo[4], hi[4]; };

struct FmDesc { const float* in; float* out; double freq_mid, freq_amp; };

struct MixChan { const float* in; double gain;  uint32_t cue; uint32_t dup;  };
struct MixDesc { const MixChan* chans; uint32_t n_ch; uint32_t pad; float* master; float* cue; };

struct OscDesc { float* mono; float* stereo; double freq; uint32_t waveform; uint32_t pad; };

struct PanDesc { const float* l; const float* r; float* out; };
struct SplitDesc { const float* in; float* l; float* r; };

struct TrigDesc { float* out; float value; uint32_t pad; };

struct PlotJob { const float* in; float* left; float* right; };

struct FirDesc { const float* in; float* out; const double* taps; float2* hist; uint32_t n_taps; uint32_t pad; };
struct ResampleDesc { const float* in; float* out; const double* taps ; float2* hist;
                      uint32_t up, down, taps_per_phase, pad; };

void launch_amplifier(const AmpDesc* d, uint32_t n, size_t frames, hipStream_t s, bool fc = false);
void launch_envelope(const EnvDesc* d, EnvState* st, uint32_t n, size_t frames, size_t fpc, const GateBits& gates, uint64_t t0, double sample_rate, hipStream_t s, bool fc = false,
                     void* scratch = nullptr, size_t scratch_bytes = 0 );
size_t envelope_scratch_bytes(uint32_t n, size_t frames);
void launch_env_ticks(const EnvTickDesc* d, uint32_t n, const GateBits& gates, uint32_t n_calls, size_t fpc, uint64_t t0, double sample_rate, EnvTick* ticks, hipStream_t s, bool fc = false);
struct EqRun { size_t frames; size_t fpc ; uint32_t n_calls; uint32_t fc ; uint64_t t0; double sr, rsr , lo_f, hi_f; const EnvTick* ticks ;
               uint32_t* started = nullptr; uint32_t started_seq = 0;
               uint32_t* env_rows = nullptr; uint32_t env_rows_seq = 0;
               uint32_t lean = 1;  };
void launch_eq_three_exact(const EqDesc* d, EqState* st, uint32_t n, const EqRun& r, void* scratch, hipStream_t s);
bool eq_use_poles_split(uint32_t n, size_t frames);
size_t eq_poles_scratch_bytes(uint32_t n, size_t frames);
int eq_scan_log2l(size_t frames);
void launch_eq_three_scan(const EqDesc* d, EqState* st, uint32_t n, const EqRun& r,
                          const EqScanTab* tabs , const EqSplit& split, const EqSpanPow& pp, hipStream_t s);
struct EqSpecPlan { uint32_t n_chunks; uint32_t chunk; uint32_t warm; uint32_t pad; uint32_t warm_hi ; };
bool eq_plan_spec(uint32_t n, size_t frames, size_t fpc, double lo_f, double hi_f, EqSpecPlan& plan, bool whole_ticks = false ,
                  bool two_tiles = false );
size_t eq_spec_scratch_bytes(uint32_t n, const EqSpecPlan& plan);
void launch_tail_gate(const uint32_t* flag, uint32_t seq, uint32_t limit_us, hipStream_t s);
int eq_epilogue_mode(uint32_t epi, uint32_t flags, bool has_ctl);
bool launch_eq_three_spec(const EqDesc* d, EqState* st, uint32_t n, const EqRun& r, const EqSpecPlan& plan, int uniform_mode ,
                          void* scratch, uint64_t* stats , hipStream_t s,
                          uint32_t* launch = nullptr ,
                          bool env_rows = true );
void eq_plan_split(uint32_t n, size_t frames, double lo_f, double hi_f, EqSplit& sp);
void launch_fm_sine(const FmDesc* d, uint32_t n, size_t frames, uint64_t t0, double sample_rate, hipStream_t s, int sin_mode );
void launch_mixer(const MixDesc* d, uint32_t n, uint32_t max_ch , size_t frames,
                  int dup_mode , hipStream_t s);
void launch_oscillator(const OscDesc* d, uint32_t n, size_t frames, uint64_t t0, double sample_rate, hipStream_t s, int sin_mode);
void launch_panner(const PanDesc* d, uint32_t n, size_t frames, hipStream_t s);
void launch_splitter(const SplitDesc* d, uint32_t n, size_t frames, hipStream_t s);
void launch_trigger(const TrigDesc* d, uint32_t n, size_t frames, size_t fpc, const GateBits* gates , hipStream_t s);
void launch_plotter(const PlotJob* d, uint32_t n, size_t spt, hipStream_t s);
void launch_f32_to_i16(const float* in, int16_t* out, size_t n, int dup, hipStream_t s);
void launch_i16_to_f32(const int16_t* in, float* out, size_t n, hipStream_t s);
struct CopyJob { void* dst; const void* src; size_t bytes; };
void launch_copy_jobs(const CopyJob* device_jobs, uint32_t n, hipStream_t s);
void launch_upload(void* dst_device, const void* src_pinned_host, size_t bytes, hipStream_t s);
struct OutState { int64_t last_clip, last_lag; uint32_t clip_status, lag_status; };
struct OutTick { uint8_t clip, clip_status, lag_status, changed; uint32_t channels; };
struct OutRun {
    const float* in; uint32_t dup;
    uint32_t frames, channels;
    int32_t left, right;
    uint32_t n_ticks;
    float* scratch; float* out;
    uint32_t* partial;
    OutState* state; OutTick* rec;
    uint64_t t0; uint32_t spt, rate, lag;
};
uint32_t out_route_blocks(size_t frames_per_tick, uint32_t channels);
void launch_output_device(const OutRun& r, hipStream_t s);
enum : uint32_t { METER_MONO = 0, METER_STEREO = 1, METER_DUP = 2 };
struct TapDesc { const float* p; uint32_t frames, layout, slot, _pad; };
struct MeterDesc { const float* p; uint32_t frames, layout, slot, hold_ticks; float release; uint32_t _pad; };
struct MeterTick { float peak[2], hold[2]; double sum_sq[2]; uint32_t over[2], frames, channels; };
struct MeterHold { float h; uint32_t a; };
struct MeterRun {
    const MeterDesc* desc; uint32_t n;
    uint32_t n_ticks, stride;
    MeterTick* rec; MeterHold* state;
};
void launch_taps(const MeterRun& r, hipStream_t s);
struct SpecRun {
    const TapDesc* desc; uint32_t n;
    uint32_t n_ticks, stride;
    uint32_t n_fft, n_bands;
    const float* window; const float2* twiddle; const uint16_t* edges;
    const float* hist_in; float* hist_out;
    float* rec;
};
void launch_taps(const SpecRun& r, hipStream_t s);
bool spectrum_tables(uint32_t n_fft, float* window, float* twiddle_re, float* twiddle_im);
static constexpr uint32_t LOUD_HIST_TICKS = 1023, LOUD_HIST_FRAMES = 11, LOUD_MAX_FRAMES = 1u << 22;
struct LoudTick { double ksq[2], momentary_sq, short_sq; float true_peak[2]; uint32_t frames, channels; };
struct LoudCoef { double bq[10], carry[16]; };
struct LoudRun {
    const TapDesc* desc; uint32_t n;
    uint32_t n_ticks, stride;
    uint32_t momentary_ticks, short_ticks;
    const LoudCoef* coef;
    const float* interp;
    double* state;
    double* walk; uint32_t walk_ticks;
    const double* ehist_in; double* ehist_out;
    const float* xhist_in; float* xhist_out;
    LoudTick* rec;
};
void launch_taps(const LoudRun& r, hipStream_t s);
bool loudness_tables(double rate, uint32_t frames, double* biquads, double* carry, float* interp);
static constexpr uint32_t STEREO_HIST_TICKS = 1023;
// ... 120 lines not shown
```

Measured before the change: 480.7 million channel-ticks/s.

## Lean envelope-row ramp math: double-double ms, clamp elision, FMA depth

Adds a lean path for the envelope-row EQ kernel. It computes milliseconds as a double-double product with a precomputed low part of 1/sr instead of the quotient-correction sequence. When no lane saturates within the tick, it skips the ramp clamp. It also uses an FMA for the amplitude depth when mod_depth has few enough mantissa bits that the FMA result stays bit-exact. All three are enabled by default via MX_EQ_RAMP_LEAN=7 and report device-side flags for debugging. The ROWS kernel's launch bounds drop occupancy from 4 to 3, and the added template variants raise code size and register pressure.

```diff
diff --git a/include/mixlab_gpu.h b/include/mixlab_gpu.h
--- a/include/mixlab_gpu.h
+++ b/include/mixlab_gpu.h
@@ -119,6 +119,7 @@
 int mx_graph_debug_eq_launch(mx_graph* g, uint32_t out[5]);
 int mx_graph_debug_eq_env_rows(mx_graph* g, uint32_t* rows);
 int mx_graph_debug_eq_lean(mx_graph* g, uint32_t* lean);
+int mx_graph_debug_eq_ramp_lean(mx_graph* g, uint32_t* forms);
 typedef struct mx_plan_node {
     int32_t pos;
     int32_t level, group;
diff --git a/mixlab_amd/abi.py b/mixlab_amd/abi.py
--- a/mixlab_amd/abi.py
+++ b/mixlab_amd/abi.py
@@ -115,6 +115,7 @@
 _proto("mx_graph_debug_eq_launch", C.c_int, C.c_void_p, C.POINTER(C.c_uint32))
 _proto("mx_graph_debug_eq_env_rows", C.c_int, C.c_void_p, C.POINTER(C.c_uint32))
 _proto("mx_graph_debug_eq_lean", C.c_int, C.c_void_p, C.POINTER(C.c_uint32))
+_proto("mx_graph_debug_eq_ramp_lean", C.c_int, C.c_void_p, C.POINTER(C.c_uint32))
 _proto("mx_graph_eq_repair_stats", C.c_int, C.c_void_p, C.POINTER(C.c_uint64))
 PLAN_NONE = 2**64 - 1
 
@@ -734,6 +735,11 @@
         check(lib.mx_graph_debug_eq_lean(self._h, C.byref(v)))
         return {"untracked": bool(v.value & 1), "unity": bool(v.value & 2)}
 
+    def debug_eq_ramp_lean(self) -> dict:
+        v = C.c_uint32()
+        check(lib.mx_graph_debug_eq_ramp_lean(self._h, C.byref(v)))
+        return {"rows": bool(v.value & 1), "noclamp": bool(v.value & 2), "depth_fma": bool(v.value & 4)}
+
     def debug_eq_records(self):
         p, n = C.c_void_p(), C.c_size_t()
         check(lib.mx_graph_debug_eq_records(self._h, C.byref(p), C.byref(n)))
diff --git a/mixlab_amd/build.py b/mixlab_amd/build.py
--- a/mixlab_amd/build.py
+++ b/mixlab_amd/build.py
@@ -23,7 +23,7 @@
 
 
 def headers() -> list[pathlib.Path]:
-    return sorted(CSRC.glob("*.hpp")) + [PKG.parent / "include" / "mixlab_gpu.h"]
+    return sorted(list(CSRC.glob("*.hpp")) + list(CSRC.glob("*.h"))) + [PKG.parent / "include" / "mixlab_gpu.h"]
 
 
 def needs_build() -> bool:
diff --git a/mixlab_amd/csrc/mx_abi.cpp b/mixlab_amd/csrc/mx_abi.cpp
--- a/mixlab_amd/csrc/mx_abi.cpp
+++ b/mixlab_amd/csrc/mx_abi.cpp
@@ -150,6 +150,10 @@
 }
 int mx_graph_debug_eq_lean(mx_graph* g, uint32_t* lean) {
     return guard([&] { REQUIRE(g && lean, "NULL argument"); *lean = g->g->eq_lean(); });
+}
+
+int mx_graph_debug_eq_ramp_lean(mx_graph* g, uint32_t* forms) {
+    return guard([&] { REQUIRE(g && forms, "NULL argument"); *forms = g->g->eq_ramp_lean(); });
 }
 
 int mx_graph_eq_repair_stats(mx_graph* g, uint64_t out[8]) {
diff --git a/mixlab_amd/csrc/mx_engine.cpp b/mixlab_amd/csrc/mx_engine.cpp
--- a/mixlab_amd/csrc/mx_engine.cpp
+++ b/mixlab_amd/csrc/mx_engine.cpp
@@ -2,6 +2,7 @@
 
 #include "mx_engine.hpp"
 #include "mx_deck.hpp"
+#include "mx_eq_ramp_lean.h"
 
 #include <cstdio>
 
@@ -108,6 +109,7 @@
     { const char* const gt = getenv("MX_TAIL_GATE_TEST"); gate_test_ = gt && atoi(gt); }
     { const char* const er = getenv("MX_EQ_ENV_ROWS"); eq_env_rows_ = !(er && atoi(er) == 0); }
     { const char* const el = getenv("MX_EQ_LEAN"); eq_lean_ = !(el && atoi(el) == 0); }
+    { const char* const rl = getenv("MX_EQ_RAMP_LEAN"); eq_ramp_lean_ = rl ? (uint32_t)atoi(rl) & 7u : 7u; }
 }
 
 void Graph::upload_eq_tables() {
@@ -376,6 +378,7 @@
                 mx_amplifier_params ap; std::memcpy(&ap, amp.params.data(), sizeof ap);
                 e.out = out_ptr(amp, 0, parity); e.ctl = in_ptr(amp, 1, true, parity);
                 e.amp_one_minus = 1.0 - ap.mod_depth; e.amp_mod_depth = ap.mod_depth; e.amp_amplitude = ap.amplitude; e.epi = 2;
+                if ((eq_ramp_lean_ & 4u) && mx_eq_depth_fma_ok(ap.mod_depth)) e.flags |= MX_EQF_DEPTH_FMA;
             } else if (nd.fuse_pan >= 0) {
                 e.out = out_ptr(nodes_[nd.fuse_pan], 0, parity); e.epi = 1;
                 if (nodes_[nd.fuse_pan].out_dup[0]) e.flags |= MX_EQF_MONO_DUP;
@@ -901,6 +904,7 @@
                         r.env_rows = (uint32_t*)eq_rows_flag_.p; r.env_rows_seq = ++eq_rows_seq_;
                     }
                     r.lean = eq_lean_ ? 1u : 0u;
+                    r.ramp_lean = (eq_ramp_lean_ & 1u) ? (eq_ramp_lean_ & 3u) : 0u; r.rsr_lo = mx_eq_rsr_lo(sample_rate_);
                     const bool opens_gate = launch_eq_three_spec((const EqDesc*)desc_of(g), (EqState*)g.state.p, n, r, plan, g.eq_mode, g.spec.p, (uint64_t*)eq_stats_.p, stream_, launch, eq_env_rows_);
                     if (!opens_gate && !gate_test_) gate_armed_ = false;
                     if (deferred_.pending) flush_deferred_tail(true);
@@ -1334,6 +1338,14 @@
     return (v[1] == eq_rows_seq_ ? 1u : 0u) | (v[2] == eq_rows_seq_ ? 2u : 0u);
 }
 
+uint32_t Graph::eq_ramp_lean() {
+    if (!eq_rows_flag_.p || !eq_rows_seq_) return 0u;
+    sync();
+    uint32_t v[6] = {0u, 0u, 0u, 0u, 0u, 0u};
+    hip_check(hipMemcpy(v, eq_rows_flag_.p, sizeof v, hipMemcpyDeviceToHost), "hipMemcpy(eq ramp lean)");
+    return (v[3] == eq_rows_seq_ ? 1u : 0u) | (v[4] == eq_rows_seq_ ? 2u : 0u) | (v[5] == eq_rows_seq_ ? 4u : 0u);
+}
+
 float* Graph::output_ptr(uint32_t node, uint32_t port, size_t* fpf, bool stream_ordered_consumer) {
     if (node >= nodes_.size() || port >= nodes_[node].out_type.size()) throw Error(MX_ERR_INVALID, "output terminal out of range");
     if (nodes_[node].out_elided[port]) throw Error(MX_ERR_INVALID, "port is not materialised: it only feeds a fused consumer (build with MX_FLAG_NO_FUSE to observe it)");
diff --git a/mixlab_amd/csrc/mx_engine.hpp b/mixlab_amd/csrc/mx_engine.hpp
--- a/mixlab_amd/csrc/mx_engine.hpp
+++ b/mixlab_amd/csrc/mx_engine.hpp
@@ -129,6 +129,7 @@
     void eq_launch(uint32_t out[5]) const { for (int k = 0; k < 5; ++k) out[k] = eq_launch_[k]; }
     bool eq_env_rows();
     uint32_t eq_lean();
+    uint32_t eq_ramp_lean();
     void set_tail_hook(std::function<void(hipStream_t)> hook) { tail_hook_ = std::move(hook); }
     void wait_before_next_run(hipEvent_t ev) { head_waits_.push_back(ev); }
     void forget_wait_before_next_run(hipEvent_t ev) { head_waits_.erase(std::remove(head_waits_.begin(), head_waits_.end(), ev), head_waits_.end()); }
@@ -226,6 +227,7 @@
     uint32_t eq_launch_[5] = {MX_EQ_LAUNCH_NONE, 0, 0, 0, 0};
     bool eq_env_rows_ = true;
     bool eq_lean_ = true;
+    uint32_t eq_ramp_lean_ = 7u;
     DevBuf eq_rows_flag_; uint32_t eq_rows_seq_ = 0;
     struct Stage { void* host = nullptr; size_t cap = 0; hipEvent_t done = nullptr; bool pending = false; };
     Stage stage_[4]; uint32_t stage_next_ = 0;
diff --git a/mixlab_amd/csrc/mx_env_math.hpp b/mixlab_amd/csrc/mx_env_math.hpp
--- a/mixlab_amd/csrc/mx_env_math.hpp
+++ b/mixlab_amd/csrc/mx_env_math.hpp
@@ -9,6 +9,9 @@
     const double r = fma(-q, sr, a);
     q = fma(r, rsr, q);
     return q * 1000.0;
+}
+__device__ __forceinline__ double ms_of_f64_dd(double a, double rsr, double rsr_lo) {
+    return __builtin_fma(a, rsr, a * rsr_lo) * 1000.0;
 }
 __device__ __forceinline__ double seq_ms(uint64_t first, uint64_t last, double sr, double rsr) {
     const uint64_t dt = last - first;
diff --git a/mixlab_amd/csrc/mx_eq_ramp_lean.h b/mixlab_amd/csrc/mx_eq_ramp_lean.h
--- /dev/null
+++ b/mixlab_amd/csrc/mx_eq_ramp_lean.h
@@ -0,0 +1,19 @@
+#ifndef MX_EQ_RAMP_LEAN_H
+#define MX_EQ_RAMP_LEAN_H
+#include <math.h>
+
+static inline double mx_eq_rsr_lo(double sr) {
+    const double y_hi = 1.0 / sr;
+    return fma(-y_hi, sr, 1.0) / sr;
+}
+
+static inline int mx_eq_depth_fma_ok(double mod_depth) {
+    if (!(mod_depth == mod_depth) || isinf(mod_depth)) return 0;
+    if (mod_depth == 0.0) return 1;
+    int e = 0;
+    const double m = frexp(fabs(mod_depth), &e);
+    if (e < -499 || e > 501) return 0;
+    const double scaled = ldexp(m, 29);
+    return scaled == floor(scaled);
+}
+#endif
diff --git a/mixlab_amd/csrc/mx_k_eq_exact.hip b/mixlab_amd/csrc/mx_k_eq_exact.hip
--- a/mixlab_amd/csrc/mx_k_eq_exact.hip
+++ b/mixlab_amd/csrc/mx_k_eq_exact.hip
@@ -119,10 +119,10 @@
     const double att = p.inv_attack * ms;
     return (float)(((PH == ENVP_ON || on) && ms < p.attack_ms) ? att : val);
 }
-template <bool FC>
+template <bool FC, bool DFMA = false >
 __device__ __forceinline__ double env_lane_depth(const EnvParams& p, const EnvLane& e, uint32_t k, double one_minus, double mod_depth, double sr, double rsr) {
     const float cc = env_lane_cc<FC>(p, e.A, e.B, e.k, e.m0, e.on != 0u, e.dt0 + k, sr, rsr);
-    return amp_depth<FC>(one_minus, mod_depth, (double)cc);
+    return amp_depth<FC || DFMA>(one_minus, mod_depth, (double)cc);
 }
 
 template <int MODE, bool STEREO, int ENVK, bool FC>
@@ -467,20 +467,20 @@
     }
 }
 
-struct EqK { double lo_f, hi_f, g_lo, g_mid, g_hi, one_minus, mod_depth, amplitude, sr, rsr; EnvParams env; };
+struct EqK { double lo_f, hi_f, g_lo, g_mid, g_hi, one_minus, mod_depth, amplitude, sr, rsr, rsr_lo ; EnvParams env; };
 __device__ __forceinline__ double pin_sgpr(double v) { asm volatile("; pinned %0" : "+s"(v)); return v; }
-__device__ __forceinline__ EqK eq_constants(const EqDesc& d, const EqRun& r) {
+__device__ __forceinline__ EqK eq_constants(const EqDesc& d, const EqRun& r, const bool rows = false ) {
     EqK k;
     k.lo_f = pin_sgpr(r.lo_f); k.hi_f = pin_sgpr(r.hi_f);
     k.g_lo = pin_sgpr(d.gain_lo); k.g_mid = pin_sgpr(d.gain_mid); k.g_hi = pin_sgpr(d.gain_hi);
     k.one_minus = pin_sgpr(d.amp_one_minus); k.mod_depth = pin_sgpr(d.amp_mod_depth); k.amplitude = pin_sgpr(d.amp_amplitude);
-    k.sr = pin_sgpr(r.sr); k.rsr = pin_sgpr(r.rsr);
+    k.sr = pin_sgpr(r.sr); k.rsr = pin_sgpr(r.rsr); k.rsr_lo = rows ? pin_sgpr(r.rsr_lo) : 0.0;
     k.env.attack_ms = pin_sgpr(d.env.attack_ms); k.env.inv_attack = pin_sgpr(d.env.inv_attack); k.env.inv_decay = pin_sgpr(d.env.inv_decay);
     k.env.sustain = pin_sgpr(d.env.sustain); k.env.one_minus_sustain = pin_sgpr(d.env.one_minus_sustain); k.env.inv_release = pin_sgpr(d.env.inv_release);
     return k;
 }
 
-template <int SB, int MODE, int ENVK, bool WARM, bool FC, bool LO_ONLY = false, bool TRACK = true, bool UNITY = false>
+template <int SB, int MODE, int ENVK, bool WARM, bool FC, bool LO_ONLY = false, bool TRACK = true, bool UNITY = false, bool DFMA = false>
 __device__ __forceinline__ void eq_tile_compute(const EqK& K, float* buf, const int lane, const int so, const int len,
                                                 const EnvTick& cur, const EnvLane& el, EqPoles& s, uint32_t& xmin, uint32_t& xmax, const float* cbuf = nullptr ) {
     const double g_lo = K.g_lo, g_mid = K.g_mid, g_hi = K.g_hi, lo_f = K.lo_f, hi_f = K.hi_f;
@@ -511,9 +511,9 @@
                         double depth;
                         const uint32_t kk = (uint32_t)(so + 4 * pce + e);
                         if (MODE == EQM_AMP_CONST) depth = depth_const;
-                        else if (MODE == EQM_AMP_CTL) depth = amp_depth<FC>(one_minus, mod_depth, (double)c4[e]);
+                        else if (MODE == EQM_AMP_CTL) depth = amp_depth<FC || DFMA>(one_minus, mod_depth, (double)c4[e]);
                         else if (ENVK == 1) depth = el.depth;
-                        else if (ENVK == 2) depth = env_lane_depth<FC>(K.env, el, kk - el.k0, one_minus, mod_depth, K.sr, K.rsr);
+                        else if (ENVK == 2) depth = env_lane_depth<FC, DFMA>(K.env, el, kk - el.k0, one_minus, mod_depth, K.sr, K.rsr);
                         else depth = env_depth<FC>(K.env, cur, one_minus, mod_depth, el.t_chunk + kk, K.sr, K.rsr);
                         v[e] = UNITY ? amp_apply_unity(y, depth) : amp_apply(y, depth, amplitude);
                     }
@@ -526,35 +526,59 @@
     }
 }
 
-struct EqEnvRow { double off_amp; uint32_t dtk ; uint32_t where ; };
+struct EqEnvRow { double off_amp; double base ; uint32_t dtk ; uint32_t where ; };
 enum { EQ_ENV_ROW_ENTRIES = 68 };
 template <typename T> __device__ __forceinline__ T* eq_uniform_ptr(T* p) {
     const uint64_t v = (uint64_t)p;
     return (T*)(((uint64_t)(uint32_t)__builtin_amdgcn_readfirstlane((int)(uint32_t)(v >> 32)) << 32) | (uint32_t)__builtin_amdgcn_readfirstlane((int)(uint32_t)v));
 }
 __device__ __forceinline__ int eq_rank64(uint64_t m) { return (int)__builtin_amdgcn_mbcnt_hi((uint32_t)(m >> 32), __builtin_amdgcn_mbcnt_lo((uint32_t)m, 0u)); }
-struct EqEnvRowPlan { int p_late, p_early, p_off; };
-__device__ __forceinline__ EqEnvRowPlan eq_env_rows_plan(const EqK& K, EqEnvRow* tab, const EnvLane& el, const bool mine, const int lane) {
+struct EqEnvRowPlan { int p_late, p_early, p_off; uint32_t lean ; };
+__device__ __forceinline__ EqEnvRowPlan eq_env_rows_plan(const EqK& K, EqEnvRow* tab, const EnvLane& el, const bool mine, const int lane, const uint32_t ramp_lean , const uint32_t n_tick) {
     const bool on = el.on != 0u;
-    const bool early = on && ms_of_u32(el.dt0, K.sr, K.rsr) < K.env.attack_ms;
+    const double ms0 = ramp_lean ? ms_of_f64_dd((double)el.dt0, K.rsr, K.rsr_lo) : ms_of_u32(el.dt0, K.sr, K.rsr);
+    const bool early = on && ms0 < K.env.attack_ms;
     const uint64_t m_late = __ballot(mine && on && !early), m_early = __ballot(mine && early), m_off = __ballot(mine && !on);
     const int n_late = __builtin_popcountll(m_late), n_early = __builtin_popcountll(m_early), n_off = __builtin_popcountll(m_off);
-    const EqEnvRowPlan plan{(n_late + 1) >> 1, (n_early + 1) >> 1, (n_off + 1) >> 1};
+    uint32_t lean = 0u;
+    if (ramp_lean) {
+        const double tt_last = el.k * (ms_of_f64_dd((double)(el.dt0 + (n_tick - 1u)), K.rsr, K.rsr_lo) - el.m0);
+        const bool sat = mine && !(tt_last < 1.0);
+        lean = 1u | (__ballot(sat && on && !early) == 0ull ? 2u : 0u) | (__ballot(sat && early) == 0ull ? 4u : 0u) | (__ballot(sat && !on) == 0ull ? 8u : 0u);
+        if (!(ramp_lean & 2u)) lean = 1u;
+    }
+    const EqEnvRowPlan plan{(n_late + 1) >> 1, (n_early + 1) >> 1, (n_off + 1) >> 1, lean};
     const int first = !on ? 2 * (plan.p_late + plan.p_early) : (early ? 2 * plan.p_late : 0);
     const int n = !on ? n_off : (early ? n_early : n_late);
     const int rank = eq_rank64(!on ? m_off : (early ? m_early : m_late));
     if (mine) {
-        const EqEnvRow e{el.B, el.dt0 - el.k0, (uint32_t)(lane * 128) | ((uint32_t)EqTileGeo<32>::sw(lane) << 4)};
+        const EqEnvRow e{el.B, (double)el.dt0 - (double)el.k0, el.dt0 - el.k0, (uint32_t)(lane * 128) | ((uint32_t)EqTileGeo<32>::sw(lane) << 4)};
         tab[first + rank] = e;
         if (rank == n - 1 && (n & 1)) tab[first + rank + 1] = e;
     }
     return plan;
 }
-template <bool FC, int PH>
-__device__ __forceinline__ const EqEnvRow* eq_env_row_passes(const EqK& K, char* cbuf, const EqEnvRow* e, const int n, const uint32_t soi, const uint32_t slot) {
+template <bool FC, int PH, bool CLAMP>
+__device__ __forceinline__ float env_row_cc(const EnvParams& p, double A, double B, double k, double m0, double a, double rsr, double rsr_lo) {
+    const double ms = ms_of_f64_dd(a, rsr, rsr_lo);
+    const double tt = k * (PH == ENVP_OFF ? ms : ms - m0);
+    const double c = CLAMP ? __builtin_fmin(tt, 1.0) : tt;
+    const double val = PH == ENVP_OFF ? B * (1.0 - c) : mul_add<FC>(B, 1.0 - c, A);
+    if (PH == ENVP_OFF || PH == ENVP_ON_LATE) return (float)val;
+    const double att = p.inv_attack * ms;
+    return (float)(ms < p.attack_ms ? att : val);
+}
+template <bool FC, int PH, int RL = 0>
+__device__ __forceinline__ const EqEnvRow* eq_env_row_passes(const EqK& K, char* cbuf, const EqEnvRow* e, const int n, const uint32_t soi, const double soid, const uint32_t slot) {
     auto pass = [&](const EqEnvRow& row) {
-        const float cc = PH == ENVP_OFF ? env_lane_cc<FC, ENVP_OFF>(K.env, 0.0, row.off_amp, K.env.inv_release, 0.0, false, row.dtk + soi, K.sr, K.rsr)
-                                        : env_lane_cc<FC, PH>(K.env, K.env.sustain, K.env.one_minus_sustain, K.env.inv_decay, K.env.attack_ms, true, row.dtk + soi, K.sr, K.rsr);
+        float cc;
+        if constexpr (RL != 0) {
+            cc = PH == ENVP_OFF ? env_row_cc<FC, ENVP_OFF, RL == 1>(K.env, 0.0, row.off_amp, K.env.inv_release, 0.0, row.base + soid, K.rsr, K.rsr_lo)
+                                : env_row_cc<FC, PH, RL == 1>(K.env, K.env.sustain, K.env.one_minus_sustain, K.env.inv_decay, K.env.attack_ms, row.base + soid, K.rsr, K.rsr_lo);
+        } else {
+            cc = PH == ENVP_OFF ? env_lane_cc<FC, ENVP_OFF>(K.env, 0.0, row.off_amp, K.env.inv_release, 0.0, false, row.dtk + soi, K.sr, K.rsr)
+                                : env_lane_cc<FC, PH>(K.env, K.env.sustain, K.env.one_minus_sustain, K.env.inv_decay, K.env.attack_ms, true, row.dtk + soi, K.sr, K.rsr);
+        }
         *reinterpret_cast<float*>(cbuf + (row.where ^ slot)) = cc;
     };
     int q = 0;
@@ -570,9 +594,17 @@
     const uint32_t soi = (uint32_t)(so + i);
     const uint32_t slot = (uint32_t)(((i >> 2) << 4) | ((i & 3) << 2));
     const EqEnvRow* e = tab + (lane >> 5);
-    e = eq_env_row_passes<FC, ENVP_ON_LATE>(K, reinterpret_cast<char*>(cbuf), e, plan.p_late, soi, slot);
-    e = eq_env_row_passes<FC, ENVP_ON>(K, reinterpret_cast<char*>(cbuf), e, plan.p_early, soi, slot);
-    eq_env_row_passes<FC, ENVP_OFF>(K, reinterpret_cast<char*>(cbuf), e, plan.p_off, soi, slot);
+    char* const cb = reinterpret_cast<char*>(cbuf);
+    if (plan.lean == 0u) {
+        e = eq_env_row_passes<FC, ENVP_ON_LATE>(K, cb, e, plan.p_late, soi, 0.0, slot);
+        e = eq_env_row_passes<FC, ENVP_ON>(K, cb, e, plan.p_early, soi, 0.0, slot);
+        eq_env_row_passes<FC, ENVP_OFF>(K, cb, e, plan.p_off, soi, 0.0, slot);
+        return;
+    }
+    const double soid = (double)soi;
+    e = (plan.lean & 2u) ? eq_env_row_passes<FC, ENVP_ON_LATE, 2>(K, cb, e, plan.p_late, soi, soid, slot) : eq_env_row_passes<FC, ENVP_ON_LATE, 1>(K, cb, e, plan.p_late, soi, soid, slot);
+    e = (plan.lean & 4u) ? eq_env_row_passes<FC, ENVP_ON, 2>(K, cb, e, plan.p_early, soi, soid, slot) : eq_env_row_passes<FC, ENVP_ON, 1>(K, cb, e, plan.p_early, soi, soid, slot);
+    if (plan.lean & 8u) eq_env_row_passes<FC, ENVP_OFF, 2>(K, cb, e, plan.p_off, soi, soid, slot); else eq_env_row_passes<FC, ENVP_OFF, 1>(K, cb, e, plan.p_off, soi, soid, slot);
 }
 
 template <int SB, int MODE, bool FC, bool OUT = true>
@@ -634,7 +666,7 @@
 
 enum { EQ_WPB = 4 };
 template <int SB, int KMODE, int KSTEREO, bool FC, int NBUF = 2, bool RT = false, bool ROWS = false >
-__global__ __launch_bounds__(64 * EQ_WPB, 4) void k_eq_three_spec_tiled(const EqDesc* __restrict__ descs, const EqState* __restrict__ states, EqRun r, EqSpecPlan plan,
+__global__ __launch_bounds__(64 * EQ_WPB, ROWS ? 3 : 4) void k_eq_three_spec_tiled(const EqDesc* __restrict__ descs, const EqState* __restrict__ states, EqRun r, EqSpecPlan plan,
                                                                          uint32_t waves_per_inst, EqChunkRec* __restrict__ recs, uint32_t n_waves) {
     extern __shared__ __attribute__((aligned(16))) float eq_tiles_all[];
     constexpr int EQ_SB = SB, EQ_TILE = EqTileGeo<SB>::TILE;
@@ -651,7 +683,7 @@
     float* const eq_tiles = eq_tiles_all + wib * EQ_WAVE_FLOATS;
     const uint32_t inst = UPTR ? (uint32_t)__builtin_amdgcn_readfirstlane((int)(wave_id / waves_per_inst)) : wave_id / waves_per_inst;
     const EqDesc& d = descs[inst];
-    const EqK K = eq_constants(d, r);
+    const EqK K = eq_constants(d, r, ROWS);
     EqTileCtx c;
     c.in = d.in; c.out = d.out;
     if constexpr (UPTR) {
@@ -779,11 +811,16 @@
         }
     } else if constexpr (KMODE == EQM_AMP_ENV) {
         const int sb_per_tick = (int)(r.fpc / EQ_SB);
-        auto lean_form = [&](const bool track, const bool unity, auto&& tick) {
-            if constexpr (!LEANK) { tick(std::true_type{}, std::false_type{}); return; }
-            if (track) { if (unity) tick(std::true_type{}, std::true_type{}); else tick(std::true_type{}, std::false_type{}); }
-            else { if (unity) tick(std::false_type{}, std::true_type{}); else tick(std::false_type{}, std::false_type{}); }
+        auto lean_form = [&](const bool track, const bool unity, const bool dfma, auto&& tick) {
+            if constexpr (!LEANK) { tick(std::true_type{}, std::false_type{}, std::false_type{}); return; }
+            auto with_depth = [&](auto TR, auto UN) {
+                if constexpr (ROWS) { if (dfma) { tick(TR, UN, std::true_type{}); return; } }
+                tick(TR, UN, std::false_type{});
+            };
+            if (track) { if (unity) with_depth(std::true_type{}, std::true_type{}); else with_depth(std::true_type{}, std::false_type{}); }
+            else { if (unity) with_depth(std::false_type{}, std::true_type{}); else with_depth(std::false_type{}, std::false_type{}); }
         };
+        const bool dfma = ROWS && !FC && (d.flags & MX_EQF_DEPTH_FMA) != 0u;
         while (g < total) {
             const int so0 = (g - n_warm) * EQ_SB;
             uint32_t jt = j;
@@ -799,8 +836,9 @@
             const bool track = !LEANK || !r.lean || __ballot(active && so0 < len && !(xmin < xmax)) != 0ull;
             const bool unity = LEANK && r.lean && K.amplitude == 1.0;
             if (envk != 3) lean_ran |= (track ? 0u : 1u) | (unity ? 2u : 0u);
+            if (envk == 2 && dfma) lean_ran |= 16u;
             if (envk == 1) {
-                lean_form(track, unity, [&](auto TR, auto UN) {
+                lean_form(track, unity, false, [&](auto TR, auto UN, auto) {
                     for (; g < g_end; ++g) { float* buf = begin_sb(g); const int so = (g - n_warm) * EQ_SB; eq_tile_compute<SB, KMODE, 1, false, FC, false, decltype(TR)::value, decltype(UN)::value>(K, buf, c.lane, so, len, cur, el, s, xmin, xmax); eq_tile_store<SB, KSTEREO != 0>(c, buf, so); }
                 });
             } else if (envk == 2) {
@@ -809,26 +847,30 @@
                     EqEnvRow* const tab = reinterpret_cast<EqEnvRow*>(eq_tiles + 2 * EQ_TILE);
                     int lt = c.lane;
                     asm volatile("; my lane %0" : "+v"(lt));
-                    const EqEnvRowPlan rows = eq_env_rows_plan(K, tab, el, active && so0 < len && el.flat == 0u, lt);
+                    const EqEnvRowPlan rows = eq_env_rows_plan(K, tab, el, active && so0 < len && el.flat == 0u, lt, r.ramp_lean, (uint32_t)r.fpc);
+                    if (rows.lean && rows.p_late + rows.p_early + rows.p_off > 0) {
+                        lean_ran |= 4u;
+                        if (((rows.lean & 2u) && rows.p_late) || ((rows.lean & 4u) && rows.p_early) || ((rows.lean & 8u) && rows.p_off)) lean_ran |= 8u;
+                    }
                     const float cc = env_lane_cc<FC>(K.env, el.A, el.B, el.k, el.m0, el.on != 0u, el.dt0, K.sr, K.rsr);
                     const f4v cc4 = {cc, cc, cc, cc};
 #pragma unroll
                     for (int q = 0; q < EQ_SB / 4; ++q) reinterpret_cast<f4v*>(cbuf + lt * EQ_SB)[q] = cc4;
                     rows_ran = true;
-                    lean_form(track, unity, [&](auto TR, auto UN) {
+                    lean_form(track, unity, dfma, [&](auto TR, auto UN, auto DF) {
                         for (; g < g_end; ++g) {
                             const int so = (g - n_warm) * EQ_SB;
                             asm volatile("s_waitcnt lgkmcnt(0)" ::: "memory");
                             eq_tile_issue<SB>(c, eq_tiles, so);
                             eq_env_rows<SB, FC>(K, cbuf, tab, rows, lt, so);
                             asm volatile("s_waitcnt vmcnt(0)" ::: "memory");
-                            eq_tile_compute<SB, EQM_AMP_CTL, 0, false, FC, false, decltype(TR)::value, decltype(UN)::value>(K, eq_tiles, c.lane, so, len, cur, el, s, xmin, xmax, cbuf);
+                            eq_tile_compute<SB, EQM_AMP_CTL, 0, false, FC, false, decltype(TR)::value, decltype(UN)::value, decltype(DF)::value>(K, eq_tiles, c.lane, so, len, cur, el, s, xmin, xmax, cbuf);
                             eq_tile_store<SB, KSTEREO != 0>(c, eq_tiles, so);
                         }
                     });
                 } else {
-                    lean_form(track, unity, [&](auto TR, auto UN) {
-                        for (; g < g_end; ++g) { float* buf = begin_sb(g); const int so = (g - n_warm) * EQ_SB; eq_tile_compute<SB, KMODE, 2, false, FC, false, decltype(TR)::value, decltype(UN)::value>(K, buf, c.lane, so, len, cur, el, s, xmin, xmax); eq_tile_store<SB, KSTEREO != 0>(c, buf, so); }
+                    lean_form(track, unity, dfma, [&](auto TR, auto UN, auto DF) {
+                        for (; g < g_end; ++g) { float* buf = begin_sb(g); const int so = (g - n_warm) * EQ_SB; eq_tile_compute<SB, KMODE, 2, false, FC, false, decltype(TR)::value, decltype(UN)::value, decltype(DF)::value>(K, buf, c.lane, so, len, cur, el, s, xmin, xmax); eq_tile_store<SB, KSTEREO != 0>(c, buf, so); }
                     });
                 }
             } else {
@@ -852,6 +894,9 @@
     if (LEANK && r.env_rows && c.lane == 0) {
         if (lean_ran & 1u) __hip_atomic_store(r.env_rows + 1, r.env_rows_seq, __ATOMIC_RELAXED, __HIP_MEMORY_SCOPE_AGENT);
         if (lean_ran & 2u) __hip_atomic_store(r.env_rows + 2, r.env_rows_seq, __ATOMIC_RELAXED, __HIP_MEMORY_SCOPE_AGENT);
+        if (lean_ran & 4u) __hip_atomic_store(r.env_rows + 3, r.env_rows_seq, __ATOMIC_RELAXED, __HIP_MEMORY_SCOPE_AGENT);
+        if (lean_ran & 8u) __hip_atomic_store(r.env_rows + 4, r.env_rows_seq, __ATOMIC_RELAXED, __HIP_MEMORY_SCOPE_AGENT);
+        if (lean_ran & 16u) __hip_atomic_store(r.env_rows + 5, r.env_rows_seq, __ATOMIC_RELAXED, __HIP_MEMORY_SCOPE_AGENT);
     }
     if (active) {
 #pragma unroll
diff --git a/mixlab_amd/csrc/mx_kernels.hpp b/mixlab_amd/csrc/mx_kernels.hpp
--- a/mixlab_amd/csrc/mx_kernels.hpp
+++ b/mixlab_amd/csrc/mx_kernels.hpp
@@ -27,7 +27,7 @@
 struct EnvTick { uint64_t seq; double off_amp; double depth; uint32_t tag; uint32_t flat; };
 struct EnvTickDesc { EnvParams p; double amp_one_minus, amp_mod_depth; EnvState* state; };
 
-enum { MX_EQF_MONO_DUP = 1u, MX_EQF_ENV = 2u };
+enum { MX_EQF_MONO_DUP = 1u, MX_EQF_ENV = 2u, MX_EQF_DEPTH_FMA = 4u };
 struct EqDesc {
     const float* in; float* out; double gain_lo, gain_mid, gain_hi;
     const float* ctl; double amp_one_minus, amp_mod_depth, amp_amplitude; uint32_t epi; uint32_t flags;
@@ -66,7 +66,8 @@
 struct EqRun { size_t frames; size_t fpc ; uint32_t n_calls; uint32_t fc ; uint64_t t0; double sr, rsr , lo_f, hi_f; const EnvTick* ticks ;
                uint32_t* started = nullptr; uint32_t started_seq = 0;
                uint32_t* env_rows = nullptr; uint32_t env_rows_seq = 0;
-               uint32_t lean = 1;  };
+               uint32_t lean = 1;
+               uint32_t ramp_lean = 0; double rsr_lo = 0.0;  };
 void launch_eq_three_exact(const EqDesc* d, EqState* st, uint32_t n, const EqRun& r, void* scratch, hipStream_t s);
 bool eq_use_poles_split(uint32_t n, size_t frames);
 size_t eq_poles_scratch_bytes(uint32_t n, size_t frames);
```

New measurement: 473.3 million channel-ticks/s. 0.985x the previous value.
